# torognes/swarm

Measured on AMD Instinct MI355X. Metric: amplicons/sec clustered (d=1), higher is better.
Workload: dtype u64; 1 GPU; 10000000 synthetic amplicons x 150 bp, d=1 (10000000 per GPU; the metric's own size; configs[1]: configs1); per_gpu_queries=10000000, db_amplicons=10000000, step=swa_d1_index_build + swa_d1_network_device (B1 seam), db and CSR resident in HBM, route=streaming (d1_stream.inc), build=local, neighbour_links=17077441

## Files before the change

swarm_amd/csrc/d1.hip:

```cpp
#include "swa_internal.h"

#include <algorithm>
#include <type_traits>
#include <cstdlib>
#include <memory>
#include <thread>

namespace {

constexpr int kWaves = 4;
constexpr int kThreads = kWaves * 64;
constexpr int kQueueCap = 128;
constexpr uint32_t kEmpty = SWA_NO_AMPLICON;
constexpr size_t kMaxZobristLds = 96 * 1024;

struct alignas(16) swa_task {
  uint64_t hash;
  uint32_t heavy;
  uint32_t code;
};

struct NetArgs {
  const uint64_t * seqs;
  const uint64_t * seq_off;
// ... 591 lines not shown
  if ((threadIdx.x & 63u) == 0u) { ssum[threadIdx.x >> 6] = sum; smax[threadIdx.x >> 6] = mx; sst0[threadIdx.x >> 6] = st0; sst1[threadIdx.x >> 6] = st1; }
  __syncthreads();
  if (threadIdx.x == 0) {
    unsigned long long s = 0, m = 0, a0 = 0, a1 = 0;
    for (int w = 0; w < 16; ++w) { s += ssum[w]; m = m > smax[w] ? m : smax[w]; a0 += sst0[w]; a1 += sst1[w]; }
    out[0] = s; out[1] = m; out[2] = a0; out[3] = a1;
  }
}

__global__ __launch_bounds__(256) void k_seg_bases(const uint32_t * __restrict__ seg_fill, uint32_t nseg,
                                                   unsigned long long * __restrict__ bases) {
  __shared__ unsigned long long part[256];
  const uint32_t chunk = (nseg + 255u) / 256u;
  const uint32_t lo = threadIdx.x * chunk, hi = min(nseg, lo + chunk);
  unsigned long long sum = 0;
  for (uint32_t i = lo; i < hi; ++i) { sum += seg_fill[i]; }
  part[threadIdx.x] = sum;
  __syncthreads();
  if (threadIdx.x == 0) {
    unsigned long long run = 0;
    for (int t = 0; t < 256; ++t) { const unsigned long long v = part[t]; part[t] = run; run += v; }
  }
  __syncthreads();
  unsigned long long at = part[threadIdx.x];
  for (uint32_t i = lo; i < hi; ++i) { bases[i] = at; at += seg_fill[i]; }
}

__global__ __launch_bounds__(256) void k_seg_compact(const uint64_t * __restrict__ edges,
                                                     const uint32_t * __restrict__ seg_fill, uint32_t nseg, uint64_t seg_cap,
                                                     const unsigned long long * __restrict__ bases,
                                                     uint64_t * __restrict__ out, uint64_t cap) {
  for (uint32_t s = blockIdx.x; s < nseg; s += gridDim.x) {
    const uint64_t fill = min((uint64_t)seg_fill[s], seg_cap);
    const uint64_t base = bases[s];
    for (uint64_t i = threadIdx.x; i < fill; i += blockDim.x) {
      if (base + i < cap) { out[base + i] = edges[(uint64_t)s * seg_cap + i]; }
    }
  }
}

#include "d1_fast.inc"
#include "d1_stream.inc"

int grid_for(const swa_ctx * ctx, uint64_t items, int per_block, int max_per_cu) {
  uint64_t blocks = (items + per_block - 1) / per_block;
  const uint64_t cap = (uint64_t)ctx->num_cus * max_per_cu;
  if (blocks > cap) { blocks = cap; }
  if (blocks < 1) { blocks = 1; }
  return (int)blocks;
}

}

void swa_warm_d1(swa_ctx * ctx) {
  hipLaunchKernelGGL(k_table_clear, dim3(1), dim3(64), 0, ctx->stream, static_cast<swa_slot *>(nullptr), (uint64_t)0,
                     static_cast<uint64_t *>(nullptr), (uint64_t)0);
}

int swa_d1_rebuild_table(swa_ctx * ctx, const uint8_t * d_is_member) {
  const uint32_t n = ctx->db.n;
  hipLaunchKernelGGL(k_table_clear, dim3(grid_for(ctx, ctx->table_size, 256, 8)), dim3(256), 0, ctx->stream,
                     static_cast<swa_slot *>(ctx->d_table.ptr), ctx->table_size,
                     static_cast<uint64_t *>(ctx->d_bloom.ptr), ctx->bloom_words);
  hipLaunchKernelGGL(k_table_insert, dim3(grid_for(ctx, n, 256, 8)), dim3(256), 0, ctx->stream,
                     static_cast<const uint64_t *>(ctx->d_seqhash.ptr), n, d_is_member,
                     static_cast<swa_slot *>(ctx->d_table.ptr), ctx->table_size - 1,
                     static_cast<unsigned long long *>(ctx->d_bloom.ptr), ctx->bloom_words - 1,
                     static_cast<const uint64_t *>(ctx->d_patterns.ptr));
  SWA_HIP(ctx, hipGetLastError());
  return SWA_OK;
}


static bool anchored_enabled() {
  const char * e = getenv("SWA_D1_PLAIN");
  return !(e != nullptr && e[0] == '1');
}

static uint32_t anchor_minlen(const swa_ctx * ctx) { return ctx->anchor_a + ctx->anchor_b + 2u * ctx->anchor_w + 1u; }

static bool anchor_applicable(const swa_ctx * ctx) {
  return anchored_enabled() && ctx->db.longest >= kMinAnchoredLen && ctx->db.longest <= 64u * kPrefetchWords * 32u - 64u;
}

static uint32_t line_quads_for(const swa_ctx * ctx) { return ctx->db.longest <= 160u ? 4u : (ctx->db.longest <= 480u ? 8u : 16u); }

static uint32_t anchor_max_nwin(const swa_ctx *) {
  uint32_t cap = 4u;
  if (const char * e = getenv("SWA_D1_ANCHOR_W")) { cap = std::min(4u, std::max(1u, (uint32_t)atoi(e) / 32u)); }
  return cap;
}
static bool windows_search_off() {
  const char * e = getenv("SWA_D1_WINDOWS");
  return e != nullptr && e[0] == '0';
}

static int ensure_db_lengths(swa_ctx * ctx) {
  if (ctx->props_ready) { return SWA_OK; }
  SWA_TRY(swa_reserve(ctx, ctx->d_rank_tmp, std::max<size_t>(ctx->d_rank_tmp.bytes, 64)));
  auto * out = static_cast<uint32_t *>(ctx->d_rank_tmp.ptr);
  SWA_HIP(ctx, hipMemsetAsync(out, 0, 8 * sizeof(uint32_t), ctx->stream));
  hipLaunchKernelGGL(k_db_lengths, dim3(grid_for(ctx, ctx->db.n, 256, 8)), dim3(256), 0, ctx->stream, ctx->db.seqlen, ctx->db.n, out);
  uint32_t host[8] = {};
  SWA_HIP(ctx, hipMemcpyAsync(host, out, sizeof(host), hipMemcpyDeviceToHost, ctx->stream));
  SWA_HIP(ctx, hipStreamSynchronize(ctx->stream));
  ctx->db_shortest = 0xFFFFFFFFu - host[0];
  for (uint32_t c = 0; c <= kWidthClasses; ++c) { ctx->class_pop[c] = host[1 + c]; }
  ctx->props_ready = true;
  return SWA_OK;
}

static ListRegions list_regions(const swa_ctx * ctx, uint64_t * total_items) {
  const uint32_t least[kListKinds] = {2, 5, 9, 17, 33, 65, kPairBigCap + 1u};
  ListRegions r{};
  uint64_t at = 0, upto = 0;
  for (uint32_t c = 0; c < kWidthClasses; ++c) {
    upto += ctx->class_pop[c];
    for (uint32_t k = 0; k < kListKinds; ++k) {
      r.at[c][k] = at;
      uint64_t room = 64;
      constexpr uint64_t per_row_tile = (tiled_item_count(kStreamGroupCap) + kStreamGroupCap / 64u - 1u) / (kStreamGroupCap / 64u);
      if (ctx->class_pop[c] != 0) { room += k + 1 < kListKinds ? std::min<uint64_t>(ctx->class_pop[c], upto / least[k]) : per_row_tile * (upto / 64 + upto / least[k]); }
      at += room;
    }
    r.at[c][kListKinds] = at;
  }
  *total_items = at;
  return r;
}

static int launch_abundance_rank(swa_ctx * ctx) {
  if (ctx->rank_ready) {
    if (ctx->db_unordered) { SWA_HIP(ctx, hipMemsetAsync(static_cast<uint32_t *>(ctx->d_flags.ptr) + 1, 1, sizeof(uint32_t), ctx->stream)); }
    return SWA_OK;
  }
  ctx->rank_ready = true;
  const uint32_t n = ctx->db.n;
  const uint32_t tiles = (n + 255u) / 256u;
  SWA_TRY(swa_reserve(ctx, ctx->d_arank, uint64_t(n) * sizeof(uint32_t)));
  SWA_TRY(swa_reserve(ctx, ctx->d_rank_tmp, uint64_t(tiles) * sizeof(uint32_t)));
  auto * rank = static_cast<uint32_t *>(ctx->d_arank.ptr);
  auto * tile_last = static_cast<uint32_t *>(ctx->d_rank_tmp.ptr);
  hipLaunchKernelGGL(k_abundance_rank, dim3(grid_for(ctx, n, 256, 8)), dim3(256), 0, ctx->stream, ctx->db.abundance, n, rank,
                     static_cast<uint32_t *>(ctx->d_flags.ptr), tile_last);
  hipLaunchKernelGGL(k_abundance_rank_carry, dim3(1), dim3(256), 0, ctx->stream, tile_last, tiles);
  hipLaunchKernelGGL(k_abundance_rank_fill, dim3(grid_for(ctx, n, 256, 8)), dim3(256), 0, ctx->stream, n, rank, tile_last);
  return SWA_OK;
}

__global__ void k_set_flags(uint32_t * flags, uint32_t unserved, uint32_t shortest_code) { flags[3] = unserved; flags[6] = shortest_code; }
__global__ void k_set_guard_made(unsigned long long * guard, uint32_t made0, uint32_t made1) { guard[0] = made0; guard[1] = made1; }

enum { kSbLines = 0, kSbRec = 1, kSbFp = 5, kSbCnt = 8, kSbTile = 10, kSbStart = 12, kSbPartial = 14, kSbScal = 16,
       kSbMembers = 17, kSbOver = 19, kSbKind = 20, kSbLinkA = 22, kSbLinkB = 23, kSbHeavy = 24, kSbMTable = 26, kSbMBloom = 27, kSbSched = 28 };

struct PartPlan { uint32_t levels; uint32_t bits[4]; uint32_t total; };
static PartPlan plan_levels(uint32_t total_bits, uint32_t max_bits = kPartMaxBits) {
  PartPlan p{};
  p.total = std::max(1u, total_bits);
  p.levels = (p.total + max_bits - 1) / max_bits;
  for (uint32_t l = 0; l < p.levels; ++l) { p.bits[l] = p.total / p.levels + (l < p.total % p.levels ? 1u : 0u); }
  return p;
}

struct PartJob {
  uint32_t nidx = 1;
  const unsigned long long * in[kMaxIdx] = {};
  unsigned long long * buf[kMaxIdx][2] = {};
  const uint64_t * cstart0[kMaxIdx] = {};
  uint64_t cstride0[kMaxIdx] = {};
  const uint32_t * csize0[kMaxIdx] = {};
  uint32_t csize_cap = 0, chunks0 = 1;
  bool single0 = true;
  uint64_t max_records = 0, max_tiles0 = 0;
  uint64_t out_cap = 0;
  uint32_t bias = 0, top_bit = 32;
  uint32_t tile = 4096;
  bool hist0_done = false;
  PartPlan plan{};
  uint32_t * out32[kMaxIdx] = {};
  uint32_t * cnt[kMaxIdx] = {}; uint32_t * ctile[kMaxIdx] = {}; uint64_t * starts[kMaxIdx] = {}; uint32_t * partial[kMaxIdx] = {};
  uint32_t * total[kMaxIdx] = {};
  uint64_t starts_stride = 0;
  const unsigned long long * out[kMaxIdx] = {}; const uint64_t * bstart[kMaxIdx] = {};
  uint32_t buckets = 0;
  int last = 0;
};

static void part_scratch(const PartJob & j, uint64_t * cnt, uint64_t * ctile, uint64_t * starts_half, uint64_t * partial) {
  uint64_t chunks = j.chunks0, c_max = 0, t_max = 0, s_max = 0;
  bool single = j.single0;
  for (uint32_t l = 0; l < j.plan.levels; ++l) {
    const uint64_t tiles = (l == 0 ? j.max_tiles0 : j.max_records / j.tile + chunks + 1);
    c_max = std::max(c_max, (tiles << j.plan.bits[l]) + 2);
    t_max = std::max(t_max, chunks + 2 + tiles + 2);
    chunks = (single ? 1 : chunks) << j.plan.bits[l];
    single = false;
    s_max = std::max(s_max, chunks + 2);
  }
  *cnt = c_max; *ctile = t_max; *starts_half = s_max; *partial = c_max / kFlatChunk + 2;
}

struct ClearList { uint32_t * p[8]; uint64_t words[8]; uint32_t n; };
__global__ __launch_bounds__(256) void k_clear_many(const ClearList c) {
  for (uint32_t k = 0; k < c.n; ++k) {
    for (uint64_t i = (uint64_t)blockIdx.x * blockDim.x + threadIdx.x; i < c.words[k]; i += (uint64_t)gridDim.x * blockDim.x) { c.p[k][i] = 0u; }
  }
}
static void clear_add(ClearList & c, void * p, uint64_t bytes) {
  c.p[c.n] = static_cast<uint32_t *>(p); c.words[c.n] = bytes / 4; ++c.n;
}
static int clear_launch(swa_ctx * ctx, const ClearList & c) {
  uint64_t most = 0;
  for (uint32_t k = 0; k < c.n; ++k) { most = std::max(most, c.words[k]); }
  if (c.n == 0 || most == 0) { return SWA_OK; }
  hipLaunchKernelGGL(k_clear_many, dim3(grid_for(ctx, most, 256, 8)), dim3(256), 0, ctx->stream, c);
  SWA_HIP(ctx, hipGetLastError());
  return SWA_OK;
}

static int run_partition(swa_ctx * ctx, PartJob & j) {
  uint64_t chunks = j.chunks0;
  bool single = j.single0;
  uint32_t used_bits = 0;
  const int cu_grid = ctx->num_cus * 8;
  for (uint32_t l = 0; l < j.plan.levels; ++l) {
    const uint32_t bits = j.plan.bits[l];
    used_bits += bits;
    const bool wide = bits > kPartMaxBits;
    const bool hist_done = l == 0 && j.hist0_done;
    const bool low_halves = l + 1 == j.plan.levels && j.out32[0] != nullptr;
    const bool have_form = wide ? (j.tile == 4096 || (j.tile == 8192 && hist_done)) && !low_halves
                                : (j.tile == 2048 && !low_halves) || j.tile == 4096;
    if (!have_form) { return swa_fail_msg(ctx, SWA_E_ARG, "partition: no kernel for this tile and bin count"); }
    PartArgs a{};
    a.single_seg = single ? 1u : 0u; a.bits = bits; a.shift = j.top_bit - used_bits; a.bias = j.bias; a.tile = j.tile;
    a.span = (single && l == 0 && chunks > 1 && j.tile == 4096 && !wide && !hist_done) ? 1u : 0u;
    const uint64_t tiles = (l == 0 ? j.max_tiles0 : j.max_records / j.tile + chunks + 1);
    a.run_bits = tiles >= (uint64_t)cu_grid ? 4u : 0u;
    for (uint32_t i = 0; i < j.nidx; ++i) {
      PartIdx & p = a.p[i];
      p.in = l == 0 ? j.in[i] : j.buf[i][(l - 1) & 1u];
      p.out = j.buf[i][l & 1u];
      p.out32 = low_halves ? j.out32[i] : nullptr;
      p.out_cap = j.out_cap;
      p.cstart = l == 0 ? j.cstart0[i] : j.starts[i] + ((l - 1) & 1u) * j.starts_stride;
      p.cstride = l == 0 ? j.cstride0[i] : 0;
      p.csize = l == 0 ? j.csize0[i] : nullptr;
      p.csize_cap = j.csize_cap;
      p.chunks = (uint32_t)chunks;
      p.ctile = j.ctile[i]; p.cnt = j.cnt[i];
      p.tchunk = j.ctile[i] + chunks + 1; p.tchunk_cap = (uint32_t)std::min<uint64_t>(tiles + 1, 0xFFFFFFFFu);
      p.next_start = j.starts[i] + (l & 1u) * j.starts_stride;
      p.total = j.total[i];
    }
    const dim3 grid_t((unsigned)((std::min<uint64_t>(std::max<uint64_t>(tiles, 1), (uint64_t)cu_grid) + 7) & ~7ull), j.nidx);
    if (chunks > 2048) { hipLaunchKernelGGL(k_part_tiles<1024>, dim3(1, j.nidx), dim3(1024), 0, ctx->stream, a); }
    else { hipLaunchKernelGGL(k_part_tiles<256>, dim3(1, j.nidx), dim3(256), 0, ctx->stream, a); }
    if (hist_done) {  }
    else if (wide) { hipLaunchKernelGGL((k_part_hist<1024, kPartTileMax, 256>), grid_t, dim3(256), 0, ctx->stream, a); }
    else if (a.span != 0u) { hipLaunchKernelGGL((k_part_hist<512, kPartTileMax, 256, true>), grid_t, dim3(256), 0, ctx->stream, a); }
    else { hipLaunchKernelGGL((k_part_hist<512, kPartTileMax, 256>), grid_t, dim3(256), 0, ctx->stream, a); }
    FlatScanArgs f{};
    f.unit_bits = bits;
    for (uint32_t i = 0; i < j.nidx; ++i) { f.v[i] = j.cnt[i]; f.units[i] = j.ctile[i] + chunks; f.partial[i] = j.partial[i]; f.total[i] = j.total[i]; }
    const dim3 grid_f((unsigned)std::min<uint64_t>(((tiles << bits) + 1 + kFlatChunk - 1) / kFlatChunk, (uint64_t)cu_grid), j.nidx);
    hipLaunchKernelGGL(k_flat_sums, grid_f, dim3(256), 0, ctx->stream, f);
    hipLaunchKernelGGL(k_flat_apply, grid_f, dim3(256), 0, ctx->stream, f);
    if (wide && j.tile == 8192) {
      constexpr size_t lds = part_scatter_lds(8192, 1024);
      if (!ctx->part_lds_opt_in) {
        SWA_HIP(ctx, hipFuncSetAttribute(reinterpret_cast<const void *>(&k_part_scatter<0, 8192, 1024, 1024>), hipFuncAttributeMaxDynamicSharedMemorySize, (int)lds));
        ctx->part_lds_opt_in = true;
      }
      hipLaunchKernelGGL((k_part_scatter<0, 8192, 1024, 1024>), grid_t, dim3(1024), lds, ctx->stream, a);
    }
    else if (wide) { hipLaunchKernelGGL((k_part_scatter<0, 4096, 1024, 512>), grid_t, dim3(512), part_scatter_lds(4096, 1024), ctx->stream, a); }
    else if (j.tile == 2048) { hipLaunchKernelGGL((k_part_scatter<0, 2048, 512, 512>), grid_t, dim3(512), part_scatter_lds(2048, 512), ctx->stream, a); }
    else if (a.span != 0u && low_halves) { hipLaunchKernelGGL((k_part_scatter<2, 4096, 512, 512, true>), grid_t, dim3(512), part_scatter_lds(4096, 512), ctx->stream, a); }
    else if (a.span != 0u) { hipLaunchKernelGGL((k_part_scatter<0, 4096, 512, 512, true>), grid_t, dim3(512), part_scatter_lds(4096, 512), ctx->stream, a); }
    else if (low_halves) { hipLaunchKernelGGL((k_part_scatter<2, 4096, 512, 512>), grid_t, dim3(512), part_scatter_lds(4096, 512), ctx->stream, a); }
    else { hipLaunchKernelGGL((k_part_scatter<0, 4096, 512, 512>), grid_t, dim3(512), part_scatter_lds(4096, 512), ctx->stream, a); }
    chunks = (single ? 1 : chunks) << bits;
    single = false;
    hipLaunchKernelGGL(k_part_starts, dim3((unsigned)std::min<uint64_t>((chunks + 256) / 256, (uint64_t)cu_grid), j.nidx), dim3(256), 0, ctx->stream, a);
    SWA_HIP(ctx, hipGetLastError());
  }
  j.buckets = (uint32_t)chunks;
  j.last = (int)((j.plan.levels - 1) & 1u);
  for (uint32_t i = 0; i < j.nidx; ++i) {
    j.out[i] = j.buf[i][j.last];
    j.bstart[i] = j.starts[i] + (uint64_t)j.last * j.starts_stride;
  }
  return SWA_OK;
}

static int ensure_lines(swa_ctx * ctx) {
  const uint32_t lq = line_quads_for(ctx);
  if (ctx->lines_ready && ctx->lines_quads == lq) { return SWA_OK; }
  const uint32_t n = ctx->db.n;
  SWA_TRY(swa_reserve(ctx, ctx->d_stream[kSbLines], (uint64_t)n * lq * 16u + 64u));
  auto * lines = static_cast<uint4 *>(ctx->d_stream[kSbLines].ptr);
  const auto * rank = static_cast<const uint32_t *>(ctx->d_arank.ptr);
  SWA_HIP(ctx, hipMemsetAsync(reinterpret_cast<uint8_t *>(lines) + (uint64_t)n * lq * 16u, 0, 64, ctx->stream));
  swa_t0(ctx, 15);
  const dim3 grid(grid_for(ctx, n, 256, 8));
  if (lq == 4u) { hipLaunchKernelGGL(k_lines_build<4>, grid, dim3(256), 0, ctx->stream, ctx->db.seqs, ctx->db.seq_off, ctx->db.seqlen, rank, n, lines); }
  else if (lq == 8u) { hipLaunchKernelGGL(k_lines_build<8>, grid, dim3(256), 0, ctx->stream, ctx->db.seqs, ctx->db.seq_off, ctx->db.seqlen, rank, n, lines); }
  else { hipLaunchKernelGGL(k_lines_build<16>, grid, dim3(256), 0, ctx->stream, ctx->db.seqs, ctx->db.seq_off, ctx->db.seqlen, rank, n, lines); }
  swa_t1(ctx, 15);
  SWA_HIP(ctx, hipGetLastError());
  ctx->lines_ready = true;
  ctx->lines_quads = lq;
  return SWA_OK;
}

static int build_stream_index(swa_ctx * ctx, uint32_t dup_first, uint32_t dup_count) {
  ctx->anchor_ready = false;
  ctx->stream_index = false;
  ctx->list_counts_ready = false;
  const uint32_t n = ctx->db.n;
  swa_lap(ctx, "(build starts)");
  SWA_TRY(ensure_db_lengths(ctx));
  swa_lap(ctx, "db lengths");
  SWA_TRY(ensure_lines(ctx));
  swa_lap(ctx, "amplicon lines");
  const uint32_t lq = ctx->lines_quads;
  uint64_t item_room = 0;
  const ListRegions regions = list_regions(ctx, &item_room);
  const bool by_rec = ctx->route_rec[0] != nullptr;
  const bool routed = ctx->route_ids[0] != nullptr || by_rec;
  const uint64_t records = routed ? std::max<uint64_t>(std::max(ctx->route_m[0], ctx->route_m[1]), 1) : n;
  const uint32_t target = kG1Target, level_bits = 10u;
  uint32_t total_bits = 1;
  while ((records >> total_bits) > target && total_bits < 3 * kPartMaxBits) { ++total_bits; }
  total_bits = std::min<uint32_t>(total_bits + ctx->stream_extra_bits, 3 * kPartMaxBits);
  const bool keys_hist = !routed;
  PartJob j;
  j.nidx = 2;
  j.plan = total_bits <= level_bits ? plan_levels(total_bits, level_bits) : plan_levels(total_bits);
  j.max_records = records;
  j.out_cap = records + 1;
  const bool one_wide_level = total_bits > kPartMaxBits && j.plan.levels == 1;
  j.tile = one_wide_level ? (keys_hist ? 8192 : 4096) : 2048;
  j.max_tiles0 = records / j.tile + 2;
  j.chunks0 = 1; j.single0 = true; j.top_bit = 32; j.bias = 0;
  uint64_t e_cnt, e_tile, e_start, e_partial;
  part_scratch(j, &e_cnt, &e_tile, &e_start, &e_partial);
  const uint64_t buckets = 1ull << total_bits;
  e_partial = std::max<uint64_t>(e_partial, ((uint64_t)kListsPerIndex * buckets + 1) / kFlatChunk + 2);
  for (int i = 0; i < 2; ++i) {
    for (int h = 0; h < 2; ++h) { SWA_TRY(swa_reserve(ctx, ctx->d_stream[kSbRec + 2 * i + h], (records + 1) * sizeof(uint64_t))); }
    SWA_TRY(swa_reserve(ctx, ctx->d_stream[kSbCnt + i], e_cnt * sizeof(uint32_t)));
    SWA_TRY(swa_reserve(ctx, ctx->d_stream[kSbTile + i], e_tile * sizeof(uint32_t)));
    SWA_TRY(swa_reserve(ctx, ctx->d_stream[kSbStart + i], (2 * e_start + 4) * sizeof(uint64_t)));
    SWA_TRY(swa_reserve(ctx, ctx->d_stream[kSbPartial + i], e_partial * sizeof(uint32_t)));
    SWA_TRY(swa_reserve(ctx, ctx->d_stream[kSbMembers + i], (records + 1) * sizeof(uint32_t)));
    SWA_TRY(swa_reserve(ctx, ctx->d_stream[kSbKind + i], ((uint64_t)kListsPerIndex * buckets + 2) * sizeof(uint32_t)));
    SWA_TRY(swa_reserve(ctx, ctx->d_aitems[i], (item_room + 1) * sizeof(swa_item)));
  }
  SWA_TRY(swa_reserve(ctx, ctx->d_stream[kSbScal], 64 * sizeof(uint64_t)));
  SWA_TRY(swa_reserve(ctx, ctx->d_stream[kSbOver], ((uint64_t)n + 8) & ~3ull));
  SWA_TRY(swa_reserve(ctx, ctx->d_acounters, kCounterWords * sizeof(uint32_t)));
  {
    ClearList c{};
    clear_add(c, ctx->d_acounters.ptr, kCounterWords * sizeof(uint32_t));
    clear_add(c, ctx->d_guard.ptr, 8 * sizeof(uint64_t));
    clear_add(c, ctx->d_stream[kSbOver].ptr, ((uint64_t)n + 8) & ~3ull);
    for (int i = 0; i < 2; ++i) { clear_add(c, static_cast<uint32_t *>(ctx->d_stream[kSbKind + i].ptr) + (uint64_t)kListsPerIndex * buckets, sizeof(uint32_t)); }
    SWA_TRY(clear_launch(ctx, c));
  }
  swa_lap(ctx, "buffers reserved, counters cleared");
  auto * dflags = static_cast<uint32_t *>(ctx->d_flags.ptr);
  auto * scal = static_cast<uint64_t *>(ctx->d_stream[kSbScal].ptr);
  const uint32_t win_a = ctx->anchor_a, win_b = ctx->anchor_b;
  const uint32_t minlen = anchor_minlen(ctx), window_mode = (win_a != 0 || win_b != 0) ? 1u : 0u;

  KeyArgs k{};
  k.lines = static_cast<const uint4 *>(ctx->d_stream[kSbLines].ptr);
  k.line_quads = lq;
  k.seqs = ctx->db.seqs; k.seq_off = ctx->db.seq_off;
  k.n = n;
  for (int i = 0; i < 2; ++i) {
    k.list[i] = routed && !by_rec ? ctx->route_ids[i] : nullptr;
    k.list_count[i] = routed ? ctx->route_m[i] : 0;
    k.rec[i] = static_cast<unsigned long long *>(ctx->d_stream[kSbRec + 2 * i + 1].ptr);
  }
  k.owner_rank = ctx->owner_rank; k.owner_world = ctx->owner_world;
  k.win_a = win_a; k.win_b = win_b; k.minlen = minlen; k.window_mode = window_mode;
  k.nwin = ctx->anchor_w / 32u;
  k.flags = dflags;
  k.guard = static_cast<unsigned long long *>(ctx->d_guard.ptr);
  k.mark_short = (!routed && ctx->owner_world == 1u) ? static_cast<uint8_t *>(ctx->d_stream[kSbOver].ptr) : nullptr;
  if (const char * e = getenv("SWA_D1_GUARD_TEST")) {
    static int builds = 0;
    const bool once = strstr(e, "-once") != nullptr;
    if (!once || builds++ == 0) { k.fault = e[0] == 'm' ? 1u : (e[0] == 'd' ? 2u : 0u); }
  }
  if (routed) {
    hipLaunchKernelGGL(k_set_flags, dim3(1), dim3(1), 0, ctx->stream, dflags,
                       ctx->db_shortest < minlen ? 1u : 0u, 0xFFFFFFFFu - ctx->db_shortest);
  }
  if (by_rec) {
    hipLaunchKernelGGL(k_set_guard_made, dim3(1), dim3(1), 0, ctx->stream, k.guard, ctx->route_m[0], ctx->route_m[1]);
  }
  swa_t0(ctx, 8);
  if (by_rec) {  }
  else if (keys_hist) {
    const uint32_t ntiles = (uint32_t)((records + j.tile - 1) / j.tile);
    for (int i = 0; i < 2; ++i) { k.hist_cnt[i] = static_cast<uint32_t *>(ctx->d_stream[kSbCnt + i].ptr); }
    k.hist_bits = j.plan.bits[0]; k.hist_tile = j.tile; k.hist_ntiles = ntiles;
    k.hist_run_bits = j.max_tiles0 >= (uint64_t)ctx->num_cus * 8 ? 4u : 0u;
    const dim3 hgrid((unsigned)((std::min<uint64_t>(ntiles, (uint64_t)ctx->num_cus * 8) + 7) & ~7ull), 1u);
    hipLaunchKernelGGL(k_keys<true>, hgrid, dim3(256), 0, ctx->stream, k);
    j.hist0_done = true;
  } else {
    const dim3 kgrid((unsigned)grid_for(ctx, records, 256, 8), routed ? 2u : 1u);
    hipLaunchKernelGGL(k_keys<false>, kgrid, dim3(256), 0, ctx->stream, k);
  }
  swa_t1(ctx, 8);
  swa_lap(ctx, "k_keys");

  for (int i = 0; i < 2; ++i) {
    j.buf[i][0] = static_cast<unsigned long long *>(ctx->d_stream[kSbRec + 2 * i].ptr);
    j.buf[i][1] = static_cast<unsigned long long *>(ctx->d_stream[kSbRec + 2 * i + 1].ptr);
    j.in[i] = by_rec ? ctx->route_rec[i] : j.buf[i][1];
    j.cstart0[i] = nullptr; j.cstride0[i] = routed ? ctx->route_m[i] : n;
    j.cnt[i] = static_cast<uint32_t *>(ctx->d_stream[kSbCnt + i].ptr);
    j.ctile[i] = static_cast<uint32_t *>(ctx->d_stream[kSbTile + i].ptr);
    j.starts[i] = static_cast<uint64_t *>(ctx->d_stream[kSbStart + i].ptr);
    j.partial[i] = static_cast<uint32_t *>(ctx->d_stream[kSbPartial + i].ptr);
    j.total[i] = reinterpret_cast<uint32_t *>(scal + 8 + i);
  }
  j.starts_stride = e_start + 2;
  swa_t0(ctx, 9);
  SWA_TRY(run_partition(ctx, j));
  swa_t1(ctx, 9);
  swa_lap(ctx, "key partition");
  if (!ctx->guard_keys_done) {
    auto * gsum = static_cast<unsigned long long *>(ctx->d_guard.ptr) + 16;
    SWA_HIP(ctx, hipMemsetAsync(gsum, 0, 8 * sizeof(uint64_t), ctx->stream));
    GuardDbArgs gd{};
    gd.seqs = ctx->db.seqs; gd.seq_off = ctx->db.seq_off; gd.seqlen = ctx->db.seqlen; gd.n = n;
    for (int i = 0; i < 2; ++i) { gd.list[i] = k.list[i]; gd.list_count[i] = routed ? ctx->route_m[i] : 0; gd.list_rec[i] = by_rec ? ctx->route_rec[i] : nullptr; }
    gd.owner_rank = k.owner_rank; gd.owner_world = k.owner_world; gd.win_a = win_a; gd.win_b = win_b; gd.nwin = k.nwin;
    gd.out = gsum;
    hipLaunchKernelGGL(k_guard_db, dim3((unsigned)grid_for(ctx, records, 256, 8), routed ? 2u : 1u), dim3(256), 0, ctx->stream, gd);
    GuardRecArgs gr{};
    for (int i = 0; i < 2; ++i) { gr.rec[i] = j.out[i]; gr.total[i] = j.total[i]; }
    gr.out = gsum + 3;
    hipLaunchKernelGGL(k_guard_records, dim3((unsigned)grid_for(ctx, records, 256, 8), 2u), dim3(256), 0, ctx->stream, gr);
    ctx->guard_keys_pending = true;
  }

  swa_lap(ctx, "guard: second opinion");
  GroupArgs g{};
  for (int i = 0; i < 2; ++i) {
    GroupIdx & x = g.g[i];
    x.rec = const_cast<unsigned long long *>(j.out[i]);
    x.bstart = j.bstart[i];
    x.buckets = j.buckets;
    x.members = static_cast<uint32_t *>(ctx->d_stream[kSbMembers + i].ptr);
    x.items_tmp = j.buf[i][j.last ^ 1];
    x.kind_cnt = static_cast<uint32_t *>(ctx->d_stream[kSbKind + i].ptr);
  }
  g.pair_big = kPairBigCap; g.group_cap = kStreamGroupCap;
  g.flags = dflags;
  g.guard = static_cast<unsigned long long *>(ctx->d_guard.ptr);
  g.over = static_cast<uint8_t *>(ctx->d_stream[kSbOver].ptr);
  swa_t0(ctx, 10);
  {
    if (!ctx->g1_lds_opt_in) {
      SWA_HIP(ctx, hipFuncSetAttribute(reinterpret_cast<const void *>(&k_group1), hipFuncAttributeMaxDynamicSharedMemorySize, (int)kG1LdsBytes));
      ctx->g1_lds_opt_in = true;
    }
    hipLaunchKernelGGL(k_group1, dim3((unsigned)std::min<uint64_t>(buckets, (uint64_t)ctx->num_cus), 2), dim3(kG1Threads), kG1LdsBytes, ctx->stream, g);
  }
  swa_t1(ctx, 10);

  FlatScanArgs f{};
  ListArgs la{};
  auto * acounters = static_cast<uint32_t *>(ctx->d_acounters.ptr);
  for (int i = 0; i < 2; ++i) {
    f.v[i] = g.g[i].kind_cnt; f.units[i] = nullptr; f.fixed[i] = (uint64_t)kListsPerIndex * buckets + 1;
    f.partial[i] = j.partial[i]; f.total[i] = reinterpret_cast<uint32_t *>(scal + 10 + i);
    ListIdx & x = la.x[i];
    x.items_tmp = g.g[i].items_tmp; x.bstart = g.g[i].bstart; x.kind_pos = g.g[i].kind_cnt; x.buckets = (uint32_t)buckets;
    x.l.items = static_cast<swa_item *>(ctx->d_aitems[i].ptr);
    x.l.region = regions;
    x.l.counters = acounters + kCounterBase + (uint32_t)i * kWidthClasses * 8u;
    x.l.pair_big = g.pair_big;
  }
  const dim3 grid_k((unsigned)std::min<uint64_t>(((uint64_t)kListsPerIndex * buckets + kFlatChunk) / kFlatChunk, (uint64_t)ctx->num_cus * 8), 2);
  hipLaunchKernelGGL(k_flat_sums, grid_k, dim3(256), 0, ctx->stream, f);
  hipLaunchKernelGGL(k_flat_apply, grid_k, dim3(256), 0, ctx->stream, f);
  hipLaunchKernelGGL(k_group_lists, dim3((unsigned)std::min<uint64_t>((buckets + 3) / 4, (uint64_t)ctx->num_cus * 8), 2), dim3(256), 0, ctx->stream, la);
  SWA_HIP(ctx, hipGetLastError());
  swa_lap(ctx, "groups + work lists");
  ctx->list_regions_items = item_room;
  ctx->anchor_ready = true;
  ctx->stream_index = true;
  ctx->guard_index = true;
  return SWA_OK;
}

static int csr_from_chunks(swa_ctx * ctx, uint32_t first, uint32_t count, const unsigned long long * links, const uint64_t * d_cstart, uint64_t cstride,
                           const uint32_t * d_csize, uint32_t chunks, uint32_t csize_cap, uint64_t max_tiles0, uint64_t link_cap,
                           uint64_t * d_offsets, uint32_t * d_neighbours, uint64_t cap) {
  uint32_t nbits = 1;
  while (nbits < 32 && ((uint64_t)1 << nbits) < count) { ++nbits; }
  uint32_t r = std::min<uint32_t>(8, nbits - 1);
  if (nbits - r > 2 * kPartMaxBits) { r = std::min<uint32_t>(kCsrMaxR, nbits - 2 * kPartMaxBits); }
  PartJob j;
  j.nidx = 1;
  j.plan = plan_levels(nbits - r);
  j.max_records = link_cap;
  j.out_cap = link_cap;
  j.tile = 4096;
  j.max_tiles0 = max_tiles0;
  j.chunks0 = chunks; j.single0 = true; j.top_bit = nbits; j.bias = first;
  j.csize_cap = csize_cap;
  uint64_t e_cnt, e_tile, e_start, e_partial;
  part_scratch(j, &e_cnt, &e_tile, &e_start, &e_partial);
  SWA_TRY(swa_reserve(ctx, ctx->d_stream[kSbLinkA], (link_cap + 1) * sizeof(uint64_t)));
  SWA_TRY(swa_reserve(ctx, ctx->d_stream[kSbLinkB], (link_cap + 1) * sizeof(uint64_t)));
  SWA_TRY(swa_reserve(ctx, ctx->d_stream[kSbCnt], e_cnt * sizeof(uint32_t)));
  SWA_TRY(swa_reserve(ctx, ctx->d_stream[kSbTile], e_tile * sizeof(uint32_t)));
  SWA_TRY(swa_reserve(ctx, ctx->d_stream[kSbStart], (2 * e_start + 4) * sizeof(uint64_t)));
  SWA_TRY(swa_reserve(ctx, ctx->d_stream[kSbPartial], e_partial * sizeof(uint32_t)));
  SWA_TRY(swa_reserve(ctx, ctx->d_stream[kSbScal], 64 * sizeof(uint64_t)));
  j.in[0] = links;
  j.buf[0][0] = static_cast<unsigned long long *>(ctx->d_stream[kSbLinkA].ptr);
  j.buf[0][1] = static_cast<unsigned long long *>(ctx->d_stream[kSbLinkB].ptr);
  j.cstart0[0] = d_cstart; j.cstride0[0] = cstride;
  j.csize0[0] = d_csize;
  j.cnt[0] = static_cast<uint32_t *>(ctx->d_stream[kSbCnt].ptr);
  j.ctile[0] = static_cast<uint32_t *>(ctx->d_stream[kSbTile].ptr);
  j.starts[0] = static_cast<uint64_t *>(ctx->d_stream[kSbStart].ptr);
  j.partial[0] = static_cast<uint32_t *>(ctx->d_stream[kSbPartial].ptr);
  auto * extra = static_cast<uint64_t *>(ctx->d_status.ptr) + 48;
  j.total[0] = reinterpret_cast<uint32_t *>(extra + 1);
  j.starts_stride = e_start + 2;
  swa_t0(ctx, 13);
  SWA_TRY(run_partition(ctx, j));
  swa_t1(ctx, 13);
  CsrArgs c{};
  c.links = j.out[0]; c.bstart = j.bstart[0]; c.buckets = j.buckets; c.r = r; c.first = first; c.count = count;
  c.offsets = d_offsets; c.neighbours = d_neighbours; c.cap = d_neighbours != nullptr ? cap : 0;
  SWA_TRY(swa_reserve(ctx, ctx->d_stream[kSbHeavy], ((uint64_t)j.buckets + 2) * sizeof(uint32_t)));
  c.heavy = static_cast<uint32_t *>(ctx->d_stream[kSbHeavy].ptr) + 1;
  c.heavy_count = static_cast<uint32_t *>(ctx->d_stream[kSbHeavy].ptr);
  c.end_copy = extra;
  SWA_HIP(ctx, hipMemsetAsync(c.heavy_count, 0, sizeof(uint32_t), ctx->stream));
  swa_t0(ctx, 14);
  static const int csr_per_cu[2] = {
    [] { int nb = 0; return hipOccupancyMaxActiveBlocksPerMultiprocessor(&nb, k_csr_bucket<8>, 256, 0) == hipSuccess && nb > 0 ? nb : 4; }(),
    [] { int nb = 0; return hipOccupancyMaxActiveBlocksPerMultiprocessor(&nb, k_csr_bucket<9>, 256, 0) == hipSuccess && nb > 0 ? nb : 4; }() };
  const dim3 cgrid((unsigned)std::min<uint64_t>(((uint64_t)j.buckets + 3) / 4, (uint64_t)ctx->num_cus * (uint64_t)csr_per_cu[r <= 8 ? 0 : 1]));
  if (r <= 8) { hipLaunchKernelGGL(k_csr_bucket<8>, cgrid, dim3(256), 0, ctx->stream, c); }
  else { hipLaunchKernelGGL(k_csr_bucket<9>, cgrid, dim3(256), 0, ctx->stream, c); }
  hipLaunchKernelGGL(k_csr_bucket_big, dim3((unsigned)ctx->num_cus * 4), dim3(256), 0, ctx->stream, c);
  swa_t1(ctx, 14);
  SWA_HIP(ctx, hipGetLastError());
  return SWA_OK;
}

static int launch_csr_stream(swa_ctx * ctx, uint32_t first, uint32_t count, uint32_t nseg, uint64_t link_cap, uint64_t * d_offsets,
                             uint32_t * d_neighbours, uint64_t cap) {
  const uint64_t tiles_per_seg = (ctx->seg_cap + 4096 - 1) / 4096;
  return csr_from_chunks(ctx, first, count, static_cast<const unsigned long long *>(ctx->d_edges.ptr), nullptr, ctx->seg_cap,
                         static_cast<const uint32_t *>(ctx->d_seg_fill.ptr), nseg, (uint32_t)std::min<uint64_t>(ctx->seg_cap, 0xFFFFFFFFu),
                         (uint64_t)nseg * tiles_per_seg + 2, link_cap, d_offsets, d_neighbours, cap);
}

#define SWA_PAIR_CASE(KERNEL, P, WW, NN) \
  if (pass == P && width == WW && nwin == NN) { hipLaunchKernelGGL((KERNEL<P, WW, NN>), dim3(grid), dim3(kThreads), 0, ctx->stream, a); return SWA_OK; }
#define SWA_PAIR_WIDTH(KERNEL, WW) \
  SWA_PAIR_CASE(KERNEL, 0, WW, 1) SWA_PAIR_CASE(KERNEL, 1, WW, 1) SWA_PAIR_CASE(KERNEL, 0, WW, 2) SWA_PAIR_CASE(KERNEL, 1, WW, 2)
#define SWA_PAIR_CASES(KERNEL) \
  SWA_PAIR_WIDTH(KERNEL, 5) SWA_PAIR_WIDTH(KERNEL, 8) SWA_PAIR_WIDTH(KERNEL, 15) SWA_PAIR_WIDTH(KERNEL, 21) \
  SWA_PAIR_CASE(KERNEL, 0, 15, 4) SWA_PAIR_CASE(KERNEL, 1, 15, 4) SWA_PAIR_CASE(KERNEL, 0, 21, 4) SWA_PAIR_CASE(KERNEL, 1, 21, 4)
#define SWA_PAIR_CASE_DYN(KERNEL, P, WW, NN) \
  if (pass == P && width == WW && nwin == NN) { \
    const int bytes = (int)PairLayout<WW>::kDynamicBytes; \
    constexpr uint32_t bit_ = 1u << (P + (WW == 21 ? 2 : 0) + (NN == 2 ? 4 : (NN == 4 ? 8 : 0))); \
    if (bytes != 0 && (ctx->pair_lds_opt_in & bit_) == 0u) {      \
      SWA_HIP(ctx, hipFuncSetAttribute(reinterpret_cast<const void *>(&KERNEL<P, WW, NN>), hipFuncAttributeMaxDynamicSharedMemorySize, bytes)); \
      ctx->pair_lds_opt_in |= bit_; \
    } \
    hipLaunchKernelGGL((KERNEL<P, WW, NN>), dim3(grid), dim3(kThreads), (size_t)bytes, ctx->stream, a); return SWA_OK; }
#define SWA_PAIR_WIDTH_DYN(KERNEL, WW) \
  SWA_PAIR_CASE_DYN(KERNEL, 0, WW, 1) SWA_PAIR_CASE_DYN(KERNEL, 1, WW, 1) SWA_PAIR_CASE_DYN(KERNEL, 0, WW, 2) SWA_PAIR_CASE_DYN(KERNEL, 1, WW, 2)
static int launch_group_pairs(swa_ctx * ctx, int pass, int width, int nwin, int grid, const AnchorArgs & a) {
  SWA_PAIR_WIDTH_DYN(k_d1_group_pairs, 5) SWA_PAIR_WIDTH_DYN(k_d1_group_pairs, 8) SWA_PAIR_WIDTH_DYN(k_d1_group_pairs, 15) SWA_PAIR_WIDTH_DYN(k_d1_group_pairs, 21)
  SWA_PAIR_CASE_DYN(k_d1_group_pairs, 0, 15, 4) SWA_PAIR_CASE_DYN(k_d1_group_pairs, 1, 15, 4) SWA_PAIR_CASE_DYN(k_d1_group_pairs, 0, 21, 4) SWA_PAIR_CASE_DYN(k_d1_group_pairs, 1, 21, 4)
  return swa_fail_msg(ctx, SWA_E_ARG, "pair kernels: no kernel for this record / window width");
}
static int launch_pairs_tiled(swa_ctx * ctx, int pass, int width, int nwin, int grid, const AnchorArgs & a) {
  SWA_PAIR_CASES(k_d1_pairs_tiled)
  return swa_fail_msg(ctx, SWA_E_ARG, "pair kernels: no kernel for this record / window width");
}

static int pair_blocks_per_cu(swa_ctx * ctx, uint32_t cls) {
  int & c = ctx->pair_blocks[cls];
  if (c == 0) {
    int nb = 0;
    const hipError_t e = cls == 0 ? hipOccupancyMaxActiveBlocksPerMultiprocessor(&nb, k_d1_group_pairs<0, 5, 1>, kThreads, 0)
                       : cls == 1 ? hipOccupancyMaxActiveBlocksPerMultiprocessor(&nb, k_d1_group_pairs<0, 8, 1>, kThreads, 0)
                       : cls == 2 ? hipOccupancyMaxActiveBlocksPerMultiprocessor(&nb, k_d1_group_pairs<0, 15, 1>, kThreads, PairLayout<15>::kDynamicBytes)
                                  : hipOccupancyMaxActiveBlocksPerMultiprocessor(&nb, k_d1_group_pairs<0, 21, 1>, kThreads, PairLayout<21>::kDynamicBytes);
    c = (e == hipSuccess && nb >= 1) ? std::min(nb, 8) : (cls <= 1u ? 4 : (cls == 2u ? 2 : 1));
  }
  return c;
}

static uint32_t seg_count(const swa_ctx * ctx) { return (uint32_t)ctx->num_cus * 8u * kWaves; }

static int launch_network_anchored(swa_ctx * ctx, int ncb, uint32_t first, uint32_t count) {
  auto * acounters = static_cast<uint32_t *>(ctx->d_acounters.ptr);
  SWA_TRY(swa_reserve(ctx, ctx->d_afallback, (2ull * count + 16) * sizeof(swa_fallback)));
  ClearList clears{};
  clear_add(clears, ctx->d_stats.ptr, 16 * sizeof(uint64_t));
  clear_add(clears, static_cast<uint64_t *>(ctx->d_guard.ptr) + 8, 8 * sizeof(uint64_t));
  clear_add(clears, acounters, kCounterBase * sizeof(uint32_t));
  clear_add(clears, ctx->d_seg_fill.ptr, 3ull * seg_count(ctx) * sizeof(uint32_t));
  uint32_t shard_bits = 6;
  while (shard_bits > 0 && (1u << shard_bits) > (uint32_t)ctx->num_cus) { --shard_bits; }
  {
    const uint64_t bytes = ((2ull * kWidthClasses) << shard_bits) * kSchedStride * sizeof(uint32_t);
    SWA_TRY(swa_reserve(ctx, ctx->d_stream[kSbSched], bytes));
    clear_add(clears, ctx->d_stream[kSbSched].ptr, bytes);
  }
  SWA_TRY(clear_launch(ctx, clears));
  const bool zlds = 4ull * ctx->zobrist_len * sizeof(uint64_t) <= kMaxZobristLds;
  const uint32_t maxwords = (ctx->db.longest + 31u) >> 5;
  swa_t0(ctx, 3);
  const bool window_mode = ctx->anchor_a != 0 || ctx->anchor_b != 0;
  uint64_t item_room = 0;
  const ListRegions regions = list_regions(ctx, &item_room);
  if (item_room != ctx->list_regions_items) { return swa_fail_msg(ctx, SWA_E_ARG, "d=1 network: the work lists in place were laid out for another database"); }
  const int nwin = (int)(ctx->anchor_w / 32u);
  for (int pass = 0; pass < 2; ++pass) {
    swa_t0(ctx, 11 + pass);
    AnchorArgs a{};
    a.pass = pass;
    a.no_cluster_breaking = ncb;
    a.first = first; a.count = count;
    a.edges = static_cast<uint64_t *>(ctx->d_edges.ptr);
    a.seg_cap = ctx->seg_cap;
    a.seg_fill = static_cast<uint32_t *>(ctx->d_seg_fill.ptr);
    a.minlen = anchor_minlen(ctx);
    a.win_word = ctx->anchor_a / 32u;
    a.win_word_b = ctx->anchor_b / 32u;
    a.window_mode = window_mode ? 1u : 0u;
    a.seg_staged = static_cast<uint32_t *>(ctx->d_seg_fill.ptr) + (uint64_t)(1 + pass) * seg_count(ctx);
    a.guard = static_cast<unsigned long long *>(ctx->d_guard.ptr);
    a.flags = static_cast<uint32_t *>(ctx->d_flags.ptr);
    a.shard_bits = shard_bits;
    a.ids = static_cast<const uint32_t *>(ctx->d_stream[kSbMembers + pass].ptr);
    a.lines = static_cast<const uint4 *>(ctx->d_stream[kSbLines].ptr);
    a.line_quads = ctx->lines_quads;
    a.pair_items = static_cast<const swa_item *>(ctx->d_aitems[pass].ptr);
    for (uint32_t cls = 0; cls < kWidthClasses; ++cls) {
      if (ctx->class_pop[cls] == 0) { continue; }
      const int width = width_words(cls);
      if (nwin == 4 && width < 15) { return swa_fail_msg(ctx, SWA_E_ARG, "pair kernels: 128-nt windows with sequences of 256 nt or less"); }
      const uint32_t pc = (uint32_t)pass * kWidthClasses + cls;
      for (uint32_t k = 0; k <= kPairClasses; ++k) { a.pair_region[k] = regions.at[cls][k]; }
      a.pair_counters = acounters + kCounterBase + pc * 8u;
      a.items = a.pair_items + regions.at[cls][kPairClasses + 1u];
      a.item_count = a.pair_counters + kPairClasses + 1u;
      a.sched_big = acounters + 8 + 2 * pc;
      a.sched_tiled = acounters + 9 + 2 * pc;
      a.sched_wide = static_cast<uint32_t *>(ctx->d_stream[kSbSched].ptr) + ((uint64_t)pc << shard_bits) * kSchedStride;
      const uint32_t * have = ctx->list_counts_ready ? ctx->list_counts + pc * 8u : nullptr;
      bool any_pairs = have == nullptr;
      for (uint32_t k = 0; k <= kPairClasses && have != nullptr; ++k) { any_pairs = any_pairs || have[k] != 0u; }
      const int pgrid = ctx->num_cus * pair_blocks_per_cu(ctx, cls);
      {
        uint64_t bundles = 0;
        for (uint32_t k = 0; k < kPairClasses && have != nullptr; ++k) { bundles += ((uint64_t)have[k] + (16u >> k) - 1u) >> (4u - k); }
        const uint64_t waves = (uint64_t)pgrid * 4u;
        a.batch = have == nullptr || bundles >= 16u * waves ? 4u : (bundles >= 8u * waves ? 2u : 1u);
      }
      if (any_pairs) { SWA_TRY(launch_group_pairs(ctx, pass, width, nwin, pgrid, a)); }
      if (have == nullptr || have[kPairClasses + 1u] != 0u) { SWA_TRY(launch_pairs_tiled(ctx, pass, width, nwin, ctx->num_cus * (cls <= 1u ? 8 : 4), a)); }
    }
    swa_t1(ctx, 11 + pass);
    SWA_HIP(ctx, hipGetLastError());
  }
  const bool use_member_table = ctx->member_index && !ctx->full_index;
  if (ctx->full_index || ctx->member_index) {
    hipLaunchKernelGGL(k_stream_fallback, dim3(grid_for(ctx, count, 256, 8)), dim3(256), 0, ctx->stream, ctx->db.seqlen, first, count,
                       static_cast<const uint8_t *>(ctx->d_stream[kSbOver].ptr), static_cast<swa_fallback *>(ctx->d_afallback.ptr), acounters + 2,
                       ctx->owner_rank, ctx->owner_world, ctx->db.seqs, ctx->db.seq_off, anchor_minlen(ctx));
  }
  NetArgs f{};
  f.seqs = ctx->db.seqs; f.seq_off = ctx->db.seq_off; f.seqlen = ctx->db.seqlen; f.abundance = ctx->db.abundance;
  f.zobrist = static_cast<const uint64_t *>(ctx->d_zobrist.ptr);
  f.zlen = ctx->zobrist_len; f.maxwords = maxwords;
  f.table = static_cast<const swa_slot *>(use_member_table ? ctx->d_stream[kSbMTable].ptr : ctx->d_table.ptr);
  f.tmask = (use_member_table ? ctx->mtable_size : ctx->table_size) - 1;
  f.bloom = static_cast<const uint64_t *>(use_member_table ? ctx->d_stream[kSbMBloom].ptr : ctx->d_bloom.ptr);
  f.bmask = (use_member_table ? ctx->mbloom_words : ctx->bloom_words) - 1;
  f.patterns = static_cast<const uint64_t *>(ctx->d_patterns.ptr);
  f.no_cluster_breaking = ncb;
  f.first = first; f.count = count;
  f.edges = static_cast<uint64_t *>(ctx->d_edges.ptr);
  f.seg_cap = ctx->seg_cap;
  f.seg_fill = static_cast<uint32_t *>(ctx->d_seg_fill.ptr);
  f.fallback = static_cast<const swa_fallback *>(ctx->d_afallback.ptr);
  f.fallback_count = acounters + 2;
  f.aux = static_cast<const swa_aux *>(ctx->d_aux.ptr);
  f.owner_rank = 0; f.owner_world = 1;
  f.window_mode = window_mode ? 1u : 0u; f.win_word = ctx->anchor_a / 32u; f.anchor_w = ctx->anchor_w;
  const size_t flds = sizeof(uint64_t) * ((zlds ? 4ull * ctx->zobrist_len : 0ull) + 1024ull +
                                          kWaves * ((size_t)(maxwords + 2u) + kQueueCap + kQueueCap / 2));
  const int fgrid = grid_for(ctx, count, kWaves, 8);
  if (!ctx->full_index && !ctx->member_index) {  }
  else if (zlds) { hipLaunchKernelGGL((k_d1_probe<true, 2>), dim3(fgrid), dim3(kThreads), flds, ctx->stream, f); }
  else { hipLaunchKernelGGL((k_d1_probe<false, 2>), dim3(fgrid), dim3(kThreads), flds, ctx->stream, f); }
  swa_t1(ctx, 3);
  SWA_HIP(ctx, hipGetLastError());
  return SWA_OK;
}
// ... 2 lines not shown
  const uint32_t n = ctx->db.n;
  ctx->zobrist_len = ctx->db.longest + 2;
  SWA_TRY(swa_reserve(ctx, ctx->d_seqhash, uint64_t(n) * sizeof(uint64_t)));
  SWA_TRY(swa_reserve(ctx, ctx->d_aux, uint64_t(n) * sizeof(swa_aux)));
  if (ctx->zobrist_resident != ctx->zobrist_len) {
    std::vector<uint64_t> zob;
    swa_zobrist_table(ctx->zobrist_len, zob);
    SWA_TRY(swa_reserve(ctx, ctx->d_zobrist, zob.size() * sizeof(uint64_t)));
    SWA_HIP(ctx, hipMemcpyAsync(ctx->d_zobrist.ptr, zob.data(), zob.size() * sizeof(uint64_t), hipMemcpyHostToDevice, ctx->stream));
    SWA_HIP(ctx, hipStreamSynchronize(ctx->stream));
    ctx->zobrist_resident = ctx->zobrist_len;
  }
  return SWA_OK;
}

static int launch_seqhash(swa_ctx * ctx, const uint8_t * only = nullptr) {
  const uint32_t n = ctx->db.n;
  const size_t zbytes = 4ull * ctx->zobrist_len * sizeof(uint64_t);
  const bool zlds = zbytes <= kMaxZobristLds;
  swa_t0(ctx, 0);
  const int hgrid = grid_for(ctx, n, 256, 8);
  if (zlds) {
    hipLaunchKernelGGL(k_seqhash<true>, dim3(hgrid), dim3(256), zbytes, ctx->stream, ctx->db.seqs, ctx->db.seq_off,
                       ctx->db.seqlen, static_cast<const uint64_t *>(ctx->d_zobrist.ptr), ctx->zobrist_len, n,
                       static_cast<uint64_t *>(ctx->d_seqhash.ptr), static_cast<swa_aux *>(ctx->d_aux.ptr), ctx->anchor_w, only);
  } else {
    hipLaunchKernelGGL(k_seqhash<false>, dim3(hgrid), dim3(256), 0, ctx->stream, ctx->db.seqs, ctx->db.seq_off,
                       ctx->db.seqlen, static_cast<const uint64_t *>(ctx->d_zobrist.ptr), ctx->zobrist_len, n,
                       static_cast<uint64_t *>(ctx->d_seqhash.ptr), static_cast<swa_aux *>(ctx->d_aux.ptr), ctx->anchor_w, only);
  }
  SWA_HIP(ctx, hipGetLastError());
  swa_t1(ctx, 0);
  return SWA_OK;
}

int swa_hash_sequences(swa_ctx * ctx) {
  SWA_TRY(prepare_hashing(ctx));
  return launch_seqhash(ctx);
}

extern "C" int swa_d1_index_build(swa_ctx * ctx, int * has_duplicates) {
  if (ctx == nullptr) { return SWA_E_ARG; }
  return swa_d1_index_build_range(ctx, 0, ctx->db.n, has_duplicates);
}

static int ensure_full_index(swa_ctx * ctx) {
  if (ctx->full_index) { return SWA_OK; }
  SWA_TRY(swa_reserve(ctx, ctx->d_table, ctx->table_size * sizeof(swa_slot)));
  SWA_TRY(swa_reserve(ctx, ctx->d_bloom, ctx->bloom_words * sizeof(uint64_t)));
  SWA_TRY(swa_hash_sequences(ctx));
  swa_t0(ctx, 1);
  SWA_TRY(swa_d1_rebuild_table(ctx, nullptr));
  swa_t1(ctx, 1);
  ctx->full_index = true;
  return SWA_OK;
}

static int choose_anchor_windows(swa_ctx * ctx) {
  ctx->anchor_a = ctx->anchor_b = 0;
  ctx->anchor_w = 32;
  SWA_TRY(ensure_db_lengths(ctx));
  const uint32_t shortest = ctx->db_shortest;
  const uint32_t n = ctx->db.n;
  const uint32_t max_nwin = anchor_max_nwin(ctx);
  ctx->anchor_w = 32u * anchor_nwin_for(shortest, 0u, max_nwin);
  if (windows_search_off()) { return SWA_OK; }
  const uint32_t stride = std::max<uint32_t>(1u, n / 65536u);
  const uint32_t samples = (n + stride - 1) / stride;
  const size_t slots = (size_t)2 * kSampleCandidates * kSampleSlots;
  SWA_TRY(swa_reserve(ctx, ctx->d_akeys[0], std::max<size_t>(ctx->d_akeys[0].bytes, slots * sizeof(uint64_t))));
  SWA_TRY(swa_reserve(ctx, ctx->d_acounts[0], std::max<size_t>(ctx->d_acounts[0].bytes, (slots + 16) * sizeof(uint32_t))));
  auto * keys = static_cast<unsigned long long *>(ctx->d_akeys[0].ptr);
  auto * counts = static_cast<uint32_t *>(ctx->d_acounts[0].ptr);
  uint32_t * stats = counts + slots;
  SWA_HIP(ctx, hipMemsetAsync(keys, 0xFF, slots * sizeof(uint64_t), ctx->stream));
  SWA_HIP(ctx, hipMemsetAsync(counts, 0, (slots + 16) * sizeof(uint32_t), ctx->stream));
  hipLaunchKernelGGL(k_anchor_sample, dim3(grid_for(ctx, samples, 256, 8)), dim3(256), 0, ctx->stream, ctx->db.seqs, ctx->db.seq_off,
                     ctx->db.seqlen, n, stride, keys, counts, stats, shortest, max_nwin);
  hipLaunchKernelGGL(k_sample_mass, dim3(grid_for(ctx, slots, 256, 8)), dim3(256), 0, ctx->stream, counts, stride, stats + 4);
  uint32_t host[8] = {};
  SWA_HIP(ctx, hipMemcpyAsync(host, stats, sizeof(host), hipMemcpyDeviceToHost, ctx->stream));
  SWA_HIP(ctx, hipStreamSynchronize(ctx->stream));
  for (uint32_t c = 0; c < kSampleCandidates; ++c) {
    const bool few_short = host[c] <= samples / 64u || c == 0;
    if (host[4 + c] <= samples / 64u && few_short) {
      ctx->anchor_a = ctx->anchor_b = 32u * c;
      ctx->anchor_w = 32u * anchor_nwin_for(shortest, 32u * c, max_nwin);
      return SWA_OK;
    }
    if (!few_short) { break; }
  }
  return SWA_OK;
}

static int ensure_anchor_windows(swa_ctx * ctx) {
  if (!ctx->windows_ready) {
    SWA_TRY(choose_anchor_windows(ctx));
    ctx->windows_chosen = ctx->anchor_a;
    ctx->windows_w = ctx->anchor_w;
    ctx->windows_ready = true;
  }
  ctx->anchor_a = ctx->anchor_b = ctx->windows_chosen;
  ctx->anchor_w = ctx->windows_w;
  return SWA_OK;
}


static int build_member_index(swa_ctx * ctx, uint32_t dup_first, uint32_t dup_count) {
  ctx->member_index = false;
  const uint32_t n = ctx->db.n;
  SWA_TRY(prepare_hashing(ctx));
  SWA_TRY(launch_seqhash(ctx, static_cast<const uint8_t *>(ctx->d_stream[kSbOver].ptr)));
  uint64_t slots = 1024;
  while (slots < 2ull * ctx->over_mass) { slots <<= 1; }
  const uint64_t words = std::max<uint64_t>(slots >> 3, 1);
  SWA_TRY(swa_reserve(ctx, ctx->d_stream[kSbMTable], slots * sizeof(swa_slot)));
  SWA_TRY(swa_reserve(ctx, ctx->d_stream[kSbMBloom], words * sizeof(uint64_t)));
  auto * table = static_cast<swa_slot *>(ctx->d_stream[kSbMTable].ptr);
  auto * bloom = static_cast<uint64_t *>(ctx->d_stream[kSbMBloom].ptr);
  swa_t0(ctx, 1);
  hipLaunchKernelGGL(k_table_clear, dim3(grid_for(ctx, slots, 256, 8)), dim3(256), 0, ctx->stream, table, slots, bloom, words);
  hipLaunchKernelGGL(k_table_insert, dim3(grid_for(ctx, n, 256, 8)), dim3(256), 0, ctx->stream, static_cast<const uint64_t *>(ctx->d_seqhash.ptr), n,
                     static_cast<const uint8_t *>(ctx->d_stream[kSbOver].ptr), table, slots - 1, reinterpret_cast<unsigned long long *>(bloom), words - 1,
                     static_cast<const uint64_t *>(ctx->d_patterns.ptr));
  swa_t1(ctx, 1);
  swa_t0(ctx, 2);
  if (dup_count != 0) {
    hipLaunchKernelGGL(k_dup_check, dim3(grid_for(ctx, dup_count, 256, 8)), dim3(256), 0, ctx->stream, ctx->db.seqs, ctx->db.seq_off, ctx->db.seqlen,
                       static_cast<const uint64_t *>(ctx->d_seqhash.ptr), dup_first, dup_count, table, slots - 1, static_cast<uint32_t *>(ctx->d_flags.ptr));
  }
  swa_t1(ctx, 2);
  SWA_HIP(ctx, hipGetLastError());
  ctx->mtable_size = slots;
  ctx->mbloom_words = words;
  ctx->member_index = true;
  return SWA_OK;
}

static int build_owned_index(swa_ctx * ctx, uint32_t first, uint32_t count, bool * needs_table, uint32_t * dups, uint32_t * oversized_mass = nullptr,
                             uint32_t * shortest = nullptr) {
  const uint32_t n = ctx->db.n;
  auto * dflags = static_cast<uint32_t *>(ctx->d_flags.ptr);
  swa_lap(ctx, "(owned index starts)");
  SWA_TRY(launch_abundance_rank(ctx));
  swa_lap(ctx, "abundance ranks");
  const uint32_t dup_first = ctx->owner_world > 1 ? 0u : first, dup_count = ctx->owner_world > 1 ? n : count;
  swa_t0(ctx, 7);
  SWA_TRY(build_stream_index(ctx, dup_first, dup_count));
  swa_t1(ctx, 7);
  auto * status = static_cast<uint32_t *>(ctx->h_status);
  SWA_HIP(ctx, hipMemcpyAsync(status, ctx->d_status.ptr, 512 * sizeof(uint32_t), hipMemcpyDeviceToHost, ctx->stream));
  SWA_HIP(ctx, hipStreamSynchronize(ctx->stream));
  const uint32_t * flags = status;
  *dups = flags[0];
  memcpy(ctx->list_counts, status + 256 + kCounterBase, sizeof(ctx->list_counts));
  ctx->list_counts_ready = true;
  if (oversized_mass != nullptr) { *oversized_mass = flags[5]; }
  if (shortest != nullptr) { *shortest = 0xFFFFFFFFu - flags[6]; }
  if (flags[2] != 0) {
    if (ctx->stream_extra_bits >= 8) { return swa_fail_msg(ctx, SWA_E_DEVICE, "streaming index build: partition still too coarse"); }
    ctx->stream_extra_bits += 2;
    SWA_HIP(ctx, hipMemsetAsync(dflags, 0, 16 * sizeof(uint32_t), ctx->stream));
    return build_owned_index(ctx, first, count, needs_table, dups, oversized_mass, shortest);
  }
  if (flags[1] != 0) { ctx->db_unordered = true; }
  *needs_table = flags[1] != 0 || flags[3] != 0 || flags[4] != 0;
  ctx->only_oversized = flags[1] == 0 && (flags[4] != 0 || flags[3] != 0) &&
                        (flags[3] == 0 || (ctx->owner_world == 1u && ctx->route_ids[0] == nullptr && ctx->route_rec[0] == nullptr));
  ctx->over_mass = flags[5];
  return SWA_OK;
}

extern "C" int swa_d1_index_build_range(swa_ctx * ctx, uint32_t first, uint32_t count, int * has_duplicates) {
  if (ctx == nullptr) { return SWA_E_ARG; }
  if (ctx->db.n == 0) { return swa_fail_msg(ctx, SWA_E_ARG, "swa_d1_index_build: no database"); }
  if (first > ctx->db.n || count > ctx->db.n - first) { return swa_fail_msg(ctx, SWA_E_ARG, "swa_d1_index_build_range: bad range"); }
  SWA_HIP(ctx, hipSetDevice(ctx->device));
  const uint32_t n = ctx->db.n;
  ctx->index_first = first; ctx->index_count = count; ctx->index_routed = ctx->route_ids[0] != nullptr || ctx->route_rec[0] != nullptr;
  ctx->d1_ready = false;
  ctx->csr_ready = false;
  ctx->anchor_ready = false;
  ctx->full_index = false;
  ctx->member_index = false;
  ctx->anchor_a = ctx->anchor_b = 0;
  for (int slot : {0, 1, 2, 7, 8, 9, 10, 15}) { ctx->ev_used[slot] = false; }
  ctx->table_size = swa_hashtable_size(n);
  const uint64_t bloom_bytes = ctx->table_size < 8 ? 8 : ctx->table_size;
  ctx->bloom_words = bloom_bytes >> 3;

  if (!ctx->patterns_resident) {
    std::vector<uint64_t> pat;
    swa_bloom_patterns(1024, 8, pat);
    SWA_TRY(swa_reserve(ctx, ctx->d_patterns, pat.size() * sizeof(uint64_t)));
    SWA_HIP(ctx, hipMemcpyAsync(ctx->d_patterns.ptr, pat.data(), pat.size() * sizeof(uint64_t), hipMemcpyHostToDevice, ctx->stream));
    SWA_HIP(ctx, hipStreamSynchronize(ctx->stream));
    ctx->patterns_resident = true;
  }
  SWA_TRY(swa_reserve(ctx, ctx->d_flags, 16 * sizeof(uint32_t)));
  SWA_TRY(swa_reserve(ctx, ctx->d_stats, 16 * sizeof(uint64_t)));
  SWA_TRY(swa_reserve(ctx, ctx->d_guard, 24 * sizeof(uint64_t)));
  SWA_HIP(ctx, hipMemsetAsync(ctx->d_status.ptr, 0, 64 + 128 + 16 * sizeof(uint64_t), ctx->stream));
  ctx->guard_index = false;
  ctx->anchor_w = 32;
  ctx->anchor_usable = anchor_applicable(ctx);

  bool owned_ok = false;
  uint32_t group_dups = 0;
  if (ctx->anchor_usable) {
    bool needs_table = false;
    uint32_t mass = 0, shortest = 0;
    swa_lap(ctx, "(index build: before the windows)");
    SWA_TRY(ensure_anchor_windows(ctx));
    swa_lap(ctx, "anchor windows");
    const uint32_t sampled = ctx->anchor_a;
    const bool routed = ctx->route_ids[0] != nullptr || ctx->route_rec[0] != nullptr;
    SWA_TRY(build_owned_index(ctx, first, count, &needs_table, &group_dups, &mass, &shortest));
    if (!routed && ctx->owner_world == 1 && needs_table && mass > n / 64u && !windows_search_off()) {
      uint32_t best = sampled, best_mass = mass;
      for (uint32_t w = sampled + 32u; 2u * w + kMinAnchoredLen <= shortest && w <= 96u; w += 32u) {
        ctx->anchor_a = ctx->anchor_b = w;
        ctx->anchor_w = 32;
        SWA_HIP(ctx, hipMemsetAsync(ctx->d_flags.ptr, 0, 16 * sizeof(uint32_t), ctx->stream));
        uint32_t m = 0;
        SWA_TRY(build_owned_index(ctx, first, count, &needs_table, &group_dups, &m));
        if (m < best_mass) { best_mass = m; best = w; }
        if (m <= n / 64u) { break; }
      }
      if (ctx->anchor_a != best) {
        ctx->anchor_a = ctx->anchor_b = best;
        ctx->anchor_w = best == sampled ? ctx->windows_w : 32u;
        SWA_HIP(ctx, hipMemsetAsync(ctx->d_flags.ptr, 0, 16 * sizeof(uint32_t), ctx->stream));
        SWA_TRY(build_owned_index(ctx, first, count, &needs_table, &group_dups));
      }
    }
    ctx->windows_chosen = ctx->anchor_a;
    ctx->windows_w = ctx->anchor_w;
    owned_ok = !needs_table;
    if (!owned_ok && ctx->only_oversized) {
      SWA_TRY(build_member_index(ctx, ctx->owner_world > 1 ? 0u : first, ctx->owner_world > 1 ? n : count));
      owned_ok = true;
      auto * mirror = static_cast<uint32_t *>(ctx->h_status);
      SWA_HIP(ctx, hipMemcpyAsync(mirror, ctx->d_flags.ptr, sizeof(uint32_t), hipMemcpyDeviceToHost, ctx->stream));
      SWA_HIP(ctx, hipStreamSynchronize(ctx->stream));
      group_dups = mirror[0];
    }
    if (!owned_ok) { SWA_HIP(ctx, hipMemsetAsync(ctx->d_flags.ptr, 0, 16 * sizeof(uint32_t), ctx->stream)); }
  }
  uint32_t flag = group_dups;
  if (!owned_ok) {
    SWA_TRY(ensure_full_index(ctx));
    swa_t0(ctx, 2);
    if (count > 0) {
      hipLaunchKernelGGL(k_dup_check, dim3(grid_for(ctx, count, 256, 8)), dim3(256), 0, ctx->stream, ctx->db.seqs, ctx->db.seq_off,
                         ctx->db.seqlen, static_cast<const uint64_t *>(ctx->d_seqhash.ptr), first, count,
                         static_cast<const swa_slot *>(ctx->d_table.ptr), ctx->table_size - 1,
                         static_cast<uint32_t *>(ctx->d_flags.ptr));
    }
    SWA_HIP(ctx, hipGetLastError());
    swa_t1(ctx, 2);
    if (ctx->anchor_usable) {
      SWA_TRY(launch_abundance_rank(ctx));
      SWA_HIP(ctx, hipGetLastError());
    }
    uint32_t flags[2] = {0, 0};
    SWA_HIP(ctx, hipMemcpyAsync(flags, ctx->d_flags.ptr, sizeof(flags), hipMemcpyDeviceToHost, ctx->stream));
    SWA_HIP(ctx, hipStreamSynchronize(ctx->stream));
    flag |= flags[0];
    if (flags[1] != 0) { ctx->anchor_usable = false; ctx->db_unordered = true; }
  }
  ctx->d1_ready = true;
  if (has_duplicates != nullptr) { *has_duplicates = flag != 0 ? 1 : 0; }
  if (flag != 0) {
    return swa_fail_msg(ctx, SWA_E_DUPLICATES, "some fasta entries have identical sequences");
  }
  return SWA_OK;
}

extern "C" uint32_t swa_d1_anchor_width(const swa_ctx * ctx) { return ctx != nullptr ? ctx->anchor_w : 0; }

extern "C" uint64_t swa_d1_table_size(const swa_ctx * ctx) { return ctx != nullptr ? ctx->table_size : 0; }

extern "C" int swa_d1_anchor_windows(const swa_ctx * ctx, uint32_t * out2) {
  if (ctx == nullptr || out2 == nullptr) { return SWA_E_ARG; }
  out2[0] = ctx->anchor_a; out2[1] = ctx->anchor_b;
  return SWA_OK;
}

static size_t network_lds_bytes(const swa_ctx * ctx, bool zlds) {
  const uint32_t maxwords = (ctx->db.longest + 31u) >> 5;
  const size_t per_wave = (size_t)(maxwords + 2u) + kQueueCap + kQueueCap / 2;
  return sizeof(uint64_t) * ((zlds ? 4ull * ctx->zobrist_len : 0ull) + 1024ull + kWaves * per_wave);
}

static int launch_network(swa_ctx * ctx, int ncb, uint32_t first, uint32_t count) {
  NetArgs a{};
  a.seqs = ctx->db.seqs; a.seq_off = ctx->db.seq_off; a.seqlen = ctx->db.seqlen; a.abundance = ctx->db.abundance;
  a.zobrist = static_cast<const uint64_t *>(ctx->d_zobrist.ptr);
  a.zlen = ctx->zobrist_len;
  a.maxwords = (ctx->db.longest + 31u) >> 5;
  a.table = static_cast<const swa_slot *>(ctx->d_table.ptr);
  a.tmask = ctx->table_size - 1;
  a.bloom = static_cast<const uint64_t *>(ctx->d_bloom.ptr);
  a.bmask = ctx->bloom_words - 1;
  a.patterns = static_cast<const uint64_t *>(ctx->d_patterns.ptr);
  a.no_cluster_breaking = ncb;
  a.first = first; a.count = count;
  a.edges = static_cast<uint64_t *>(ctx->d_edges.ptr);
  a.seg_cap = ctx->seg_cap;
  a.seg_fill = static_cast<uint32_t *>(ctx->d_seg_fill.ptr);
  a.owner_rank = ctx->owner_rank; a.owner_world = ctx->owner_world;
  a.anchor_w = 32;
  SWA_HIP(ctx, hipMemsetAsync(ctx->d_stats.ptr, 0, 16 * sizeof(uint64_t), ctx->stream));
  const bool zlds = 4ull * ctx->zobrist_len * sizeof(uint64_t) <= kMaxZobristLds;
  const size_t lds = network_lds_bytes(ctx, zlds);
  const int grid = grid_for(ctx, count, kWaves, 8);
  swa_t0(ctx, 3);
  if (zlds) { hipLaunchKernelGGL((k_d1_probe<true, 0>), dim3(grid), dim3(kThreads), lds, ctx->stream, a); }
  else { hipLaunchKernelGGL((k_d1_probe<false, 0>), dim3(grid), dim3(kThreads), lds, ctx->stream, a); }
  swa_t1(ctx, 3);
  SWA_HIP(ctx, hipGetLastError());
  return SWA_OK;
}

static int guard_check(swa_ctx * ctx, const uint64_t * g, const uint64_t * got) {
  char msg[256];
  if (g[10] != 0) {
    snprintf(msg, sizeof(msg), "d=1 guard: %llu member(s) filed under an anchor key that is not theirs", (unsigned long long)g[10]);
    return swa_fail_msg(ctx, SWA_E_INTERNAL, msg);
  }
  if (ctx->stream_index && ctx->guard_keys_pending) {
    ctx->guard_keys_pending = false;
    for (int i = 0; i < 2; ++i) {
      if (g[16 + i] != g[19 + i]) {
        snprintf(msg, sizeof(msg), "d=1 guard: the %s derived from the amplicon lines are not the ones the packed database gives (%016llx / %016llx)",
                 i == 0 ? "prefix-side key records" : "suffix-side key records", (unsigned long long)g[19 + i],
                 (unsigned long long)g[16 + i]);
        return swa_fail_msg(ctx, SWA_E_INTERNAL, msg);
      }
    }
    ctx->guard_keys_done = true;
  }
  if (ctx->stream_index && ctx->guard_index) {
    for (int i = 0; i < 2; ++i) {
      if (g[i] != g[2 + i] + g[4 + i] + g[6 + i]) {
        snprintf(msg, sizeof(msg), "d=1 guard: index %d has %llu key records but %llu + %llu + %llu grouped members", i, (unsigned long long)g[i],
                 (unsigned long long)g[2 + i], (unsigned long long)g[4 + i], (unsigned long long)g[6 + i]);
        return swa_fail_msg(ctx, SWA_E_INTERNAL, msg);
      }
      if (got[2 + i] != g[2 + i]) {
        snprintf(msg, sizeof(msg), "d=1 guard: pass %d staged %llu members of %llu listed", i, (unsigned long long)got[2 + i], (unsigned long long)g[2 + i]);
        return swa_fail_msg(ctx, SWA_E_INTERNAL, msg);
      }
    }
  }
  return SWA_OK;
}
static int csr_check(swa_ctx * ctx, uint64_t csr_end, uint32_t links_sorted, uint64_t n_edges) {
  if (csr_end != n_edges || (uint64_t)links_sorted != (n_edges & 0xFFFFFFFFull)) {
    char msg[256];
    snprintf(msg, sizeof(msg), "d=1 guard: %llu links found, %u sorted, CSR ends at %llu", (unsigned long long)n_edges, links_sorted, (unsigned long long)csr_end);
    return swa_fail_msg(ctx, SWA_E_INTERNAL, msg);
  }
  return SWA_OK;
}

static int network_run(swa_ctx * ctx, int no_cluster_breaking, uint32_t first, uint32_t count, uint64_t * d_offsets,
                       uint32_t * d_neighbours, uint64_t * d_edge_list, uint64_t cap, uint64_t * total) {
  SWA_HIP(ctx, hipSetDevice(ctx->device));
  const uint32_t nseg = (uint32_t)ctx->num_cus * 8u * kWaves;
  SWA_TRY(swa_reserve(ctx, ctx->d_seg_fill, 3ull * nseg * sizeof(uint32_t)));
  SWA_TRY(swa_reserve(ctx, ctx->d_guard, 24 * sizeof(uint64_t)));
  if (ctx->seg_cap == 0) {
    ctx->seg_cap = 512;
    while (ctx->seg_cap < 8ull * count / nseg) { ctx->seg_cap <<= 1; }
    const char * env_cap = getenv("SWA_D1_SEG_CAP");
    if (env_cap != nullptr && atoi(env_cap) > 0) { ctx->seg_cap = (uint64_t)atoi(env_cap); }
  }
  uint64_t n_edges = 0;
  uint64_t stream_link_cap = 0;
  bool clean = false;
  bool twins = false;
  for (int attempt = 0; attempt < 8 && !clean; ++attempt) {
    SWA_TRY(swa_reserve(ctx, ctx->d_edges, uint64_t(nseg) * ctx->seg_cap * sizeof(uint64_t)));
    if (!ctx->anchor_usable) { SWA_HIP(ctx, hipMemsetAsync(ctx->d_seg_fill.ptr, 0, 3ull * nseg * sizeof(uint32_t), ctx->stream)); }
    if (ctx->anchor_usable) {
      if (!(ctx->anchor_ready && ctx->stream_index)) {
        swa_t0(ctx, 7);
        SWA_TRY(launch_abundance_rank(ctx));
        SWA_HIP(ctx, hipMemsetAsync(static_cast<uint32_t *>(ctx->d_flags.ptr) + 2, 0, 5 * sizeof(uint32_t), ctx->stream));
        SWA_TRY(build_stream_index(ctx, 0, 0));
        swa_t1(ctx, 7);
        if (!ctx->full_index) {
          uint32_t fl[6] = {};
          SWA_HIP(ctx, hipMemcpyAsync(fl, ctx->d_flags.ptr, sizeof(fl), hipMemcpyDeviceToHost, ctx->stream));
          SWA_HIP(ctx, hipStreamSynchronize(ctx->stream));
          ctx->member_index = false;
          if (fl[3] != 0 || fl[4] != 0) { SWA_TRY(ensure_full_index(ctx)); }
        }
      }
      SWA_TRY(launch_network_anchored(ctx, no_cluster_breaking, first, count));
    }
    else {
      SWA_TRY(ensure_full_index(ctx));
      SWA_TRY(launch_network(ctx, no_cluster_breaking, first, count));
    }
    hipLaunchKernelGGL(k_seg_reduce, dim3(1), dim3(1024), 0, ctx->stream, static_cast<const uint32_t *>(ctx->d_seg_fill.ptr),
                       nseg, static_cast<unsigned long long *>(ctx->d_stats.ptr) + 8);
    const bool check_unserved = ctx->anchor_usable && !ctx->full_index && !ctx->member_index;
    swa_t0(ctx, 4);
    if (d_edge_list != nullptr) {
      SWA_TRY(swa_reserve(ctx, ctx->d_seg_base, uint64_t(nseg) * sizeof(uint64_t)));
      hipLaunchKernelGGL(k_seg_bases, dim3(1), dim3(256), 0, ctx->stream, static_cast<const uint32_t *>(ctx->d_seg_fill.ptr), nseg,
                         static_cast<unsigned long long *>(ctx->d_seg_base.ptr));
      hipLaunchKernelGGL(k_seg_compact, dim3(std::min<uint32_t>(nseg, (uint32_t)ctx->num_cus * 8u)), dim3(256), 0, ctx->stream,
                         static_cast<const uint64_t *>(ctx->d_edges.ptr), static_cast<const uint32_t *>(ctx->d_seg_fill.ptr),
                         nseg, ctx->seg_cap, static_cast<const unsigned long long *>(ctx->d_seg_base.ptr), d_edge_list, cap);
    } else {
      stream_link_cap = std::max<uint64_t>(std::max<uint64_t>(cap, stream_link_cap), 2ull * count + 1024);
      SWA_TRY(launch_csr_stream(ctx, first, count, nseg, stream_link_cap, d_offsets, d_neighbours, cap));
    }
    SWA_HIP(ctx, hipGetLastError());
    swa_t1(ctx, 4);
    auto * status = static_cast<uint64_t *>(ctx->h_status);
    SWA_HIP(ctx, hipMemcpyAsync(status, ctx->d_status.ptr, 64 * sizeof(uint64_t), hipMemcpyDeviceToHost, ctx->stream));
    uint32_t * unserved_at = reinterpret_cast<uint32_t *>(status + 64);
    *unserved_at = 0;
    if (check_unserved) {
      SWA_HIP(ctx, hipMemcpyAsync(unserved_at, static_cast<uint32_t *>(ctx->d_acounters.ptr) + 2, sizeof(uint32_t), hipMemcpyDeviceToHost, ctx->stream));
    }
    SWA_HIP(ctx, hipStreamSynchronize(ctx->stream));
    const uint32_t unserved = *unserved_at;
    const uint64_t * got = status + 8 + 8;
    const uint64_t * guard = status + 24;
    const uint32_t anchor_overflow = reinterpret_cast<const uint32_t *>(status)[2];
    const uint64_t csr_end = status[48];
    const uint32_t links_sorted = (uint32_t)status[49];
    const bool guarded = ctx->anchor_usable;
    n_edges = got[0];
    if (guarded && anchor_overflow != 0) {
      ctx->stream_extra_bits = std::min<uint32_t>(ctx->stream_extra_bits + 2, 8);
      ctx->anchor_ready = false;
      continue;
    }
    if (check_unserved && unserved != 0) {
      SWA_TRY(ensure_full_index(ctx));
      continue;
    }
    if (d_edge_list == nullptr && got[1] <= ctx->seg_cap && n_edges > stream_link_cap) {
      stream_link_cap = n_edges + 1024;
      continue;
    }
    if (got[1] <= ctx->seg_cap) {
      clean = true;
      if (guarded) { SWA_TRY(guard_check(ctx, guard, got)); }
      if (d_edge_list == nullptr) { SWA_TRY(csr_check(ctx, csr_end, links_sorted, n_edges)); }
      twins = guarded && reinterpret_cast<const uint32_t *>(status)[0] != 0u;
      break;
    }
    while (ctx->seg_cap < 2 * got[1]) { ctx->seg_cap <<= 1; }
  }
  if (!clean) {
    return swa_fail_msg(ctx, SWA_E_DEVICE, "swa_d1_network: per-wave link segments still overflowed after 8 attempts");
  }
  *total = n_edges;
  if (twins) { return swa_fail_msg(ctx, SWA_E_DUPLICATES, "some fasta entries have identical sequences"); }
  if (n_edges > cap) { return swa_fail_msg(ctx, SWA_E_CAPACITY, "swa_d1_network: neighbour buffer too small"); }
  return SWA_OK;
}

static int network_run_guarded(swa_ctx * ctx, int no_cluster_breaking, uint32_t first, uint32_t count, uint64_t * d_offsets,
                               uint32_t * d_neighbours, uint64_t * d_edge_list, uint64_t cap, uint64_t * total) {
  const int rc = network_run(ctx, no_cluster_breaking, first, count, d_offsets, d_neighbours, d_edge_list, cap, total);
  if (rc != SWA_E_INTERNAL || ctx->index_routed) { return rc; }
  const std::string first_msg = ctx->err;
  fprintf(stderr, "swarm-amd: %s; rebuilding the index from the packed database and repeating the step\n", first_msg.c_str());
  ++ctx->guard_retries;
  ctx->lines_ready = ctx->props_ready = ctx->windows_ready = ctx->rank_ready = false;
  ctx->anchor_ready = ctx->stream_index = ctx->member_index = ctx->full_index = false;
  ctx->guard_index = ctx->guard_keys_done = ctx->guard_keys_pending = false;
  ctx->stream_extra_bits = 0;
  int dup = 0;
  const int rb = swa_d1_index_build_range(ctx, ctx->index_first, ctx->index_count, &dup);
  if (rb != SWA_OK && rb != SWA_E_DUPLICATES) { return rb; }
  const int again = network_run(ctx, no_cluster_breaking, first, count, d_offsets, d_neighbours, d_edge_list, cap, total);
  if (again == SWA_E_INTERNAL) { ctx->err = first_msg + "; after a rebuild: " + ctx->err; }
  return again;
}

extern "C" int swa_d1_guard_retries(const swa_ctx * ctx) { return ctx != nullptr ? (int)ctx->guard_retries : 0; }

extern "C" int swa_d1_network_device(swa_ctx * ctx, int no_cluster_breaking, uint32_t first, uint32_t count,
                                     uint64_t * d_offsets, uint32_t * d_neighbours, uint64_t cap, uint64_t * total) {
  if (ctx == nullptr) { return SWA_E_ARG; }
  if (!ctx->d1_ready) { return swa_fail_msg(ctx, SWA_E_ARG, "swa_d1_network: call swa_d1_index_build first"); }
  if (count == 0 || (uint64_t)first + count > ctx->db.n || d_offsets == nullptr || total == nullptr ||
      (d_neighbours == nullptr && cap != 0)) {
    return swa_fail_msg(ctx, SWA_E_ARG, "swa_d1_network: bad range or null buffer");
  }
  return network_run_guarded(ctx, no_cluster_breaking, first, count, d_offsets, d_neighbours, nullptr, cap, total);
}

extern "C" int swa_d1_network_edges_device(swa_ctx * ctx, int no_cluster_breaking, uint32_t first, uint32_t count,
                                           uint64_t * d_edge_list, uint64_t cap, uint64_t * total) {
  if (ctx == nullptr) { return SWA_E_ARG; }
  if (!ctx->d1_ready) { return swa_fail_msg(ctx, SWA_E_ARG, "swa_d1_network: call swa_d1_index_build first"); }
  if (count == 0 || (uint64_t)first + count > ctx->db.n || d_edge_list == nullptr || total == nullptr) {
    return swa_fail_msg(ctx, SWA_E_ARG, "swa_d1_network_edges: bad range or null buffer");
  }
  return network_run_guarded(ctx, no_cluster_breaking, first, count, nullptr, nullptr, d_edge_list, cap, total);
}

int swa_d1_csr_from_lists(swa_ctx * ctx, const unsigned long long * d_links, const uint64_t * starts, const uint64_t * counts, uint32_t lists,
                          uint64_t * d_offsets, uint32_t * d_neighbours, uint64_t cap) {
  SWA_HIP(ctx, hipSetDevice(ctx->device));
  const uint32_t n = ctx->db.n;
  uint64_t all = 0, tiles = 2;
  std::vector<uint64_t> h_start(lists);
  std::vector<uint32_t> h_size(lists);
  for (uint32_t r = 0; r < lists; ++r) {
    if (counts[r] > 0xFFFFFFFFull) { return swa_fail_msg(ctx, SWA_E_CAPACITY, "swa_d1_csr_from_lists: a list of more than 2^32 links"); }
    h_start[r] = starts[r]; h_size[r] = (uint32_t)counts[r];
    all += counts[r]; tiles += (counts[r] + 4095) / 4096;
  }
  SWA_TRY(swa_reserve(ctx, ctx->d_seg_base, ((uint64_t)lists * 3 / 2 + 2) * sizeof(uint64_t)));
  auto * d_start = static_cast<uint64_t *>(ctx->d_seg_base.ptr);
  auto * d_size = reinterpret_cast<uint32_t *>(d_start + lists);
  SWA_HIP(ctx, hipMemcpyAsync(d_start, h_start.data(), lists * sizeof(uint64_t), hipMemcpyHostToDevice, ctx->stream));
  SWA_HIP(ctx, hipMemcpyAsync(d_size, h_size.data(), lists * sizeof(uint32_t), hipMemcpyHostToDevice, ctx->stream));
  SWA_HIP(ctx, hipStreamSynchronize(ctx->stream));
  return csr_from_chunks(ctx, 0, n, d_links, d_start, 0, d_size, lists, 0xFFFFFFFFu, tiles, all + 1, d_offsets, d_neighbours, cap);
}

extern "C" int swa_d1_route_slice(swa_ctx * ctx, uint32_t first, uint32_t count, uint32_t world, uint32_t * d_ids, uint64_t cap,
                                  uint32_t * d_counts) {
  if (ctx == nullptr) { return SWA_E_ARG; }
  if (ctx->db.n == 0) { return swa_fail_msg(ctx, SWA_E_ARG, "swa_d1_route_slice: no database"); }
  if (first > ctx->db.n || count > ctx->db.n - first) { return swa_fail_msg(ctx, SWA_E_ARG, "swa_d1_route_slice: bad range"); }
  if (world == 0 || world > kRouteMaxWorld || d_ids == nullptr || d_counts == nullptr || cap == 0) {
    return swa_fail_msg(ctx, SWA_E_ARG, "swa_d1_route_slice: bad argument (1..64 ranks)");
  }
  SWA_HIP(ctx, hipSetDevice(ctx->device));
  SWA_TRY(swa_reserve(ctx, ctx->d_flags, 16 * sizeof(uint32_t)));
  SWA_TRY(ensure_anchor_windows(ctx));
  SWA_HIP(ctx, hipMemsetAsync(d_counts, 0, (2ull * world + 1) * sizeof(uint32_t), ctx->stream));
  if (count != 0) {
    hipLaunchKernelGGL(k_anchor_route, dim3(grid_for(ctx, (count + kRoutePerThread - 1) / kRoutePerThread, 256, 8)), dim3(256), 0, ctx->stream,
                       ctx->db.seqs, ctx->db.seq_off, ctx->db.seqlen, first, count, world, ctx->anchor_a, ctx->anchor_b, ctx->anchor_w / 32u, d_ids, cap,
                       d_counts);
  }
  SWA_HIP(ctx, hipGetLastError());
  SWA_HIP(ctx, hipStreamSynchronize(ctx->stream));
  return SWA_OK;
}

extern "C" int swa_d1_index_build_routed(swa_ctx * ctx, const uint32_t * d_ids_prefix, uint32_t n_prefix, const uint32_t * d_ids_suffix,
                                         uint32_t n_suffix, int * has_duplicates) {
  if (ctx == nullptr) { return SWA_E_ARG; }
  if (ctx->db.n == 0) { return swa_fail_msg(ctx, SWA_E_ARG, "swa_d1_index_build_routed: no database"); }
  if (ctx->owner_world <= 1) { return swa_fail_msg(ctx, SWA_E_ARG, "swa_d1_index_build_routed: call swa_d1_set_ownership(rank, world > 1) first"); }
  if ((n_prefix != 0 && d_ids_prefix == nullptr) || (n_suffix != 0 && d_ids_suffix == nullptr)) { return swa_fail_msg(ctx, SWA_E_ARG, "swa_d1_index_build_routed: null list"); }
  SWA_HIP(ctx, hipSetDevice(ctx->device));
  SWA_TRY(ensure_db_lengths(ctx));
  static const uint32_t nothing = 0;
  ctx->route_ids[0] = n_prefix != 0 ? d_ids_prefix : &nothing; ctx->route_m[0] = n_prefix;
  ctx->route_ids[1] = n_suffix != 0 ? d_ids_suffix : &nothing; ctx->route_m[1] = n_suffix;
  const int rc = swa_d1_index_build_range(ctx, 0, ctx->db.n, has_duplicates);
  ctx->route_ids[0] = ctx->route_ids[1] = nullptr;
  ctx->route_m[0] = ctx->route_m[1] = 0;
  return rc;
}

extern "C" int swa_d1_route_slice_records(swa_ctx * ctx, uint32_t first, uint32_t count, uint32_t world, uint64_t * d_records, uint64_t cap,
                                          uint32_t * d_counts) {
  if (ctx == nullptr) { return SWA_E_ARG; }
  if (ctx->db.n == 0) { return swa_fail_msg(ctx, SWA_E_ARG, "swa_d1_route_slice_records: no database"); }
  if (first > ctx->db.n || count > ctx->db.n - first) { return swa_fail_msg(ctx, SWA_E_ARG, "swa_d1_route_slice_records: bad range"); }
  if (world == 0 || world > kRouteMaxWorld || d_records == nullptr || d_counts == nullptr || cap == 0) {
    return swa_fail_msg(ctx, SWA_E_ARG, "swa_d1_route_slice_records: bad argument (1..64 ranks)");
  }
  SWA_HIP(ctx, hipSetDevice(ctx->device));
  SWA_TRY(swa_reserve(ctx, ctx->d_flags, 16 * sizeof(uint32_t)));
  SWA_TRY(ensure_anchor_windows(ctx));
  SWA_HIP(ctx, hipMemsetAsync(d_counts, 0, (2ull * world + 1) * sizeof(uint32_t), ctx->stream));
  if (count != 0) {
    hipLaunchKernelGGL(k_anchor_route_records, dim3(grid_for(ctx, (count + 3) / 4, 256, 8)), dim3(256), 0, ctx->stream,
                       ctx->db.seqs, ctx->db.seq_off, ctx->db.seqlen, first, count, world, ctx->anchor_a, ctx->anchor_b, ctx->anchor_w / 32u,
                       reinterpret_cast<unsigned long long *>(d_records), cap, d_counts);
  }
  SWA_HIP(ctx, hipGetLastError());
// ... 437 lines not shown
```

swarm_amd/csrc/d1_stream.inc:

```

constexpr uint32_t kPartTileMax = 4096;
constexpr uint32_t kPartMaxBits = 9;
constexpr unsigned long long kRecAbsent = ~0ull;
constexpr uint32_t kMaxIdx = 2;
constexpr uint32_t kStreamGroupCap = 4096;

template <int LQ>
__global__ __launch_bounds__(256) void k_lines_build(const uint64_t * __restrict__ seqs, const uint64_t * __restrict__ seq_off,
                                                     const uint32_t * __restrict__ seqlen, const uint32_t * __restrict__ rank, uint32_t n,
                                                     uint4 * __restrict__ lines) {
  constexpr uint32_t C = 2u * LQ - 1u;
  for (uint32_t i = blockIdx.x * blockDim.x + threadIdx.x; i < n; i += gridDim.x * blockDim.x) {
    const uint32_t len = seqlen[i];
    const uint64_t * s = seqs + seq_off[i];
    const uint32_t nw = (len + 31u) >> 5;
    uint32_t d[4 * LQ];
    d[0] = len; d[1] = rank[i];
#pragma unroll
    for (uint32_t k = 0; k < C; ++k) {
      const uint64_t w = k < nw ? s[k] : 0ull;
      d[2 + 2 * k] = (uint32_t)w; d[3 + 2 * k] = (uint32_t)(w >> 32);
    }
#pragma unroll
    for (uint32_t q = 0; q < (uint32_t)LQ; ++q) { lines[(uint64_t)i * LQ + q] = make_uint4(d[4 * q], d[4 * q + 1], d[4 * q + 2], d[4 * q + 3]); }
// ... 285 lines not shown
    for (uint32_t k = 0; k < 8u; ++k) {
      const uint32_t c = base + threadIdx.x * 8u + k;
      v[k] = c < p.chunks ? (a.span != 0u ? part_chunk_size(p, c) : (part_chunk_size(p, c) + a.tile - 1u) / a.tile) : 0u;
    }
#pragma unroll
    for (uint32_t k = 0; k < 8u; ++k) { mine += v[k]; }
    uint64_t total;
    uint64_t run = carry + block_exclusive_scan_of<THREADS>(mine, smem, total);
#pragma unroll
    for (uint32_t k = 0; k < 8u; ++k) {
      const uint32_t c = base + threadIdx.x * 8u + k;
      if (c < p.chunks) {
        p.ctile[c] = (uint32_t)run;
        if (v[k] != 0u && a.span != 0u) {
          const uint32_t r32 = (uint32_t)run;
          const uint32_t first = tile_pow2 ? (r32 + a.tile - 1u) >> tile_shift : (r32 + a.tile - 1u) / a.tile;
          const uint32_t n = (tile_pow2 ? (r32 + v[k] + a.tile - 1u) >> tile_shift : (r32 + v[k] + a.tile - 1u) / a.tile) - first;
          if (n <= 4u) {
#pragma unroll
            for (uint32_t i = 0; i < 4u; ++i) { if (i < n && first + i < p.tchunk_cap) { p.tchunk[first + i] = c; } }
          }
        }
      }
      run += v[k];
    }
    carry += total;
  }
  if (threadIdx.x == 0) {
    if (a.span != 0u) { carry = ((uint32_t)carry + a.tile - 1u) / a.tile; }
    p.ctile[p.chunks] = (uint32_t)carry;
    p.cnt[carry << a.bits] = 0u;
  }
}

__device__ __forceinline__ uint32_t part_chunk_of(const uint32_t * ctile, uint32_t chunks, uint32_t t) {
  uint32_t lo = 0, hi = chunks;
  while (lo < hi) { const uint32_t mid = (lo + hi) >> 1; if (ctile[mid] <= t) { lo = mid + 1u; } else { hi = mid; } }
  return lo - 1u;
}

__device__ __forceinline__ uint64_t part_flat(const PartArgs & a, const PartIdx & p, uint32_t c, uint32_t t, uint32_t b) {
  if (a.single_seg != 0u) { return (uint64_t)b * p.ctile[p.chunks] + t; }
  const uint32_t t0 = p.ctile[c], nt = p.ctile[c + 1] - t0;
  return ((uint64_t)t0 << a.bits) + (uint64_t)b * nt + (t - t0);
}

struct PartTile { uint32_t c, count; uint64_t first; };

__device__ __forceinline__ PartTile part_tile(const PartIdx & p, uint32_t tile_records, uint32_t t, uint32_t * sh) {
  if (threadIdx.x == 0) {
    sh[0] = part_chunk_of(p.ctile, p.chunks, t);
  }
  __syncthreads();
  PartTile r;
  r.c = sh[0];
  const uint32_t within = (t - p.ctile[r.c]) * tile_records;
  r.first = (p.cstart != nullptr ? p.cstart[r.c] : (p.csize != nullptr ? (uint64_t)r.c * p.cstride : 0ull)) + within;
  r.count = min(tile_records, part_chunk_size(p, r.c) - within);
  return r;
}

constexpr uint32_t kSpanFast = 4;
constexpr uint32_t kSpanRound = 256;
struct SpanLds { uint32_t c_lo, n, count, q0; uint64_t shift[kSpanFast]; uint32_t before[kSpanRound + 1]; };
__device__ __forceinline__ uint64_t part_chunk_base(const PartIdx & p, uint32_t c) {
  return p.cstart != nullptr ? p.cstart[c] : (p.csize != nullptr ? (uint64_t)c * p.cstride : 0ull);
}
template <uint32_t PER, uint32_t THREADS, typename Take>
__device__ __forceinline__ uint32_t part_span(const PartIdx & p, uint32_t tile_records, uint32_t t, SpanLds & s, Take take) {
  if (threadIdx.x == 0) {
    const uint32_t last = p.chunks - 1u;
    const uint32_t total = p.ctile[last] + part_chunk_size(p, last);
    const uint32_t q0 = t * tile_records, q1 = min(q0 + tile_records, total) - 1u;
    const auto chunk_at = [&](uint32_t tile, uint32_t q) -> uint32_t {
      const uint32_t c = tile < p.tchunk_cap ? p.tchunk[tile] : 0xFFFFFFFFu;
      if (c < p.chunks && p.ctile[c] <= q && q < (c + 1u < p.chunks ? p.ctile[c + 1u] : total)) { return c; }
      return part_chunk_of(p.ctile, p.chunks, q);
    };
    const uint32_t c_lo = chunk_at(t, q0);
    const uint32_t c_hi = q1 + 1u < total ? chunk_at(t + 1u, q1 + 1u) : part_chunk_of(p.ctile, p.chunks, q1);
    s.c_lo = c_lo; s.n = c_hi - c_lo + 1u; s.count = q1 - q0 + 1u; s.q0 = q0;
  }
  __syncthreads();
  const uint32_t n = s.n, count = s.count, q0 = s.q0, c_lo = s.c_lo;
  if (n <= kSpanFast) {
    if (threadIdx.x < n) {
      const uint32_t before = p.ctile[c_lo + threadIdx.x];
      s.before[threadIdx.x] = before;
      s.shift[threadIdx.x] = part_chunk_base(p, c_lo + threadIdx.x) - before;
    }
    __syncthreads();
    const uint32_t b1 = n > 1u ? s.before[1] : 0xFFFFFFFFu, b2 = n > 2u ? s.before[2] : 0xFFFFFFFFu, b3 = n > 3u ? s.before[3] : 0xFFFFFFFFu;
#pragma unroll
    for (uint32_t k = 0; k < PER; ++k) {
      const uint32_t j = k * THREADS + threadIdx.x, q = q0 + j;
      const uint32_t i = (q >= b1 ? 1u : 0u) + (q >= b2 ? 1u : 0u) + (q >= b3 ? 1u : 0u);
      if (j < count) { take(k, s.shift[i] + q); }
    }
    return count;
  }
  for (uint32_t r0 = 0; r0 < n; r0 += kSpanRound) {
    const uint32_t m = min(kSpanRound, n - r0);
    if (r0 != 0u) { __syncthreads(); }
    for (uint32_t i = threadIdx.x; i <= m; i += THREADS) { s.before[i] = r0 + i < n ? p.ctile[c_lo + r0 + i] : 0xFFFFFFFFu; }
    __syncthreads();
    const uint32_t from = s.before[0], upto = s.before[m];
#pragma unroll
    for (uint32_t k = 0; k < PER; ++k) {
      const uint32_t j = k * THREADS + threadIdx.x, q = q0 + j;
      if (j < count && q >= from && q < upto) {
        uint32_t lo = 0, hi = m;
        while (lo < hi) { const uint32_t mid = (lo + hi) >> 1; if (s.before[mid] <= q) { lo = mid + 1u; } else { hi = mid; } }
        take(k, part_chunk_base(p, c_lo + r0 + lo - 1u) + (q - s.before[lo - 1u]));
      }
    }
  }
  return count;
}

template <uint32_t BINS, uint32_t TILE, uint32_t THREADS, bool SPAN = false>
__global__ __launch_bounds__(THREADS) void k_part_hist(const PartArgs a) {
  __shared__ uint32_t hist[BINS];
  __shared__ uint32_t sh[1];
  __shared__ typename std::conditional<SPAN, SpanLds, uint32_t>::type span;
  const PartIdx & p = a.p[blockIdx.y];
  const uint32_t bins = 1u << a.bits;
  const uint32_t ntiles = p.ctile[p.chunks];
  for (uint32_t v = blockIdx.x; v < ((ntiles + (8u << a.run_bits) - 1u) & ~((8u << a.run_bits) - 1u)); v += gridDim.x) {
    const uint32_t t = xcd_tile(v, a.run_bits);
    if (t >= ntiles) { continue; }
    for (uint32_t b = threadIdx.x; b < bins; b += THREADS) { hist[b] = 0u; }
    PartTile tile{0u, 0u, 0ull};
    const auto count_one = [&](unsigned long long r) {
      if (r != kRecAbsent) { atomicAdd(&hist[(((uint32_t)(r >> 32) - a.bias) >> a.shift) & (bins - 1u)], 1u); }
    };
    if constexpr (SPAN) {
      (void)part_span<TILE / THREADS, THREADS>(p, a.tile, t, span, [&](uint32_t, uint64_t place) { count_one(p.in[place]); });
    } else {
      tile = part_tile(p, a.tile, t, sh);
#pragma unroll
      for (uint32_t k = 0; k < TILE / THREADS; ++k) {
        const uint32_t j = k * THREADS + threadIdx.x;
        if (j < tile.count) { count_one(p.in[tile.first + j]); }
      }
    }
    __syncthreads();
    for (uint32_t b = threadIdx.x; b < bins; b += THREADS) { p.cnt[part_flat(a, p, tile.c, t, b)] = hist[b]; }
    __syncthreads();
  }
}

constexpr uint32_t kFlatChunk = 4096;
constexpr uint32_t kFlatPer = kFlatChunk / 256u;
struct FlatScanArgs { uint32_t * v[kMaxIdx]; const uint32_t * units[kMaxIdx]; uint32_t unit_bits; uint64_t fixed[kMaxIdx]; uint32_t * partial[kMaxIdx]; uint32_t * total[kMaxIdx]; };
__device__ __forceinline__ uint64_t flat_length(const FlatScanArgs & a, uint32_t i) {
  return a.units[i] != nullptr ? ((uint64_t)*a.units[i] << a.unit_bits) + 1u : a.fixed[i];
}

__global__ __launch_bounds__(256) void k_flat_sums(const FlatScanArgs a) {
  __shared__ uint64_t smem[4];
  const uint32_t * v = a.v[blockIdx.y];
  const uint64_t m = flat_length(a, blockIdx.y);
  for (uint64_t blk = blockIdx.x; blk * kFlatChunk < m; blk += gridDim.x) {
    const uint64_t base = blk * kFlatChunk + (uint64_t)threadIdx.x * kFlatPer;
    uint64_t s = 0;
#pragma unroll
    for (uint32_t k = 0; k < kFlatPer; ++k) { if (base + k < m) { s += v[base + k]; } }
    uint64_t total;
    (void)block_exclusive_scan(s, smem, total);
    if (threadIdx.x == 0) { a.partial[blockIdx.y][blk] = (uint32_t)total; }
  }
}

__global__ __launch_bounds__(256) void k_flat_apply(const FlatScanArgs a) {
  __shared__ uint64_t smem[4];
  uint32_t * v = a.v[blockIdx.y];
  const uint64_t m = flat_length(a, blockIdx.y);
  const uint32_t * partial = a.partial[blockIdx.y];
  const uint64_t nblk = (m + kFlatChunk - 1) / kFlatChunk;
  for (uint64_t blk = blockIdx.x; blk < nblk; blk += gridDim.x) {
    uint64_t before = 0;
    for (uint64_t q = threadIdx.x; q < blk; q += 256u) { before += partial[q]; }
    uint64_t prefix;
    (void)block_exclusive_scan(before, smem, prefix);
    const uint64_t base = blk * kFlatChunk + (uint64_t)threadIdx.x * kFlatPer;
    uint32_t c[kFlatPer];
    uint64_t s = 0;
#pragma unroll
    for (uint32_t k = 0; k < kFlatPer; ++k) { c[k] = base + k < m ? v[base + k] : 0u; s += c[k]; }
    uint64_t total;
    uint64_t run = prefix + block_exclusive_scan(s, smem, total);
#pragma unroll
    for (uint32_t k = 0; k < kFlatPer; ++k) { if (base + k < m) { v[base + k] = (uint32_t)run; } run += c[k]; }
    if (blk + 1 == nblk && threadIdx.x == 0) { *a.total[blockIdx.y] = (uint32_t)(prefix + total); }
  }
}

template <uint32_t THREADS>
__device__ __forceinline__ uint64_t block_exclusive_scan_of(uint64_t v, uint64_t * smem, uint64_t & total) {
  const uint32_t lane = threadIdx.x & 63u, wave = threadIdx.x >> 6;
  uint64_t incl = v;
#pragma unroll
  for (unsigned d = 1; d < 64; d <<= 1) { const uint64_t t = swa_shfl_up_u64(incl, d); if (lane >= d) { incl += t; } }
  if (lane == 63u) { smem[wave] = incl; }
  __syncthreads();
  uint64_t wave_off = 0, tot = 0;
#pragma unroll
  for (uint32_t w = 0; w < THREADS / 64u; ++w) { const uint64_t x = smem[w]; wave_off += w < wave ? x : 0ull; tot += x; }
  __syncthreads();
  total = tot;
  return wave_off + incl - v;
}

template <int MODE, uint32_t TILE, uint32_t BINS, uint32_t THREADS, bool SPAN = false>
__global__ __launch_bounds__(THREADS) __attribute__((amdgpu_waves_per_eu(SPAN && THREADS == 512 ? 8 : 1))) void k_part_scatter(const PartArgs a) {
  constexpr uint32_t kPartPer = TILE / THREADS;
  extern __shared__ __attribute__((aligned(16))) unsigned long long part_lds[];
  unsigned long long * stage = part_lds;
  uint32_t * hist = reinterpret_cast<uint32_t *>(stage + TILE);
  uint32_t * lstart = hist + BINS;
  uint32_t * goff = lstart + BINS;
  __shared__ uint64_t smem[THREADS / 64u];
  __shared__ uint32_t sh[1];
  __shared__ typename std::conditional<SPAN, SpanLds, uint32_t>::type span;
  const PartIdx & p = a.p[blockIdx.y];
  const uint32_t bins = 1u << a.bits;
  const uint32_t ntiles = p.ctile[p.chunks];
  for (uint32_t v = blockIdx.x; v < ((ntiles + (8u << a.run_bits) - 1u) & ~((8u << a.run_bits) - 1u)); v += gridDim.x) {
    const uint32_t t = xcd_tile(v, a.run_bits);
    if (t >= ntiles) { continue; }
    for (uint32_t b = threadIdx.x; b < bins; b += THREADS) { hist[b] = 0u; }
    PartTile tile{0u, 0u, 0ull};
    unsigned long long rec[kPartPer];
    uint32_t pos[kPartPer];
    const auto digit_of = [&](unsigned long long r) { return (((uint32_t)(r >> 32) - a.bias) >> a.shift) & (bins - 1u); };
    if constexpr (SPAN) {
#pragma unroll
      for (uint32_t k = 0; k < kPartPer; ++k) { rec[k] = kRecAbsent; pos[k] = 0u; }
      (void)part_span<kPartPer, THREADS>(p, TILE, t, span, [&](uint32_t k, uint64_t place) {
        rec[k] = p.in[place];
        if (rec[k] != kRecAbsent) { pos[k] = atomicAdd(&hist[digit_of(rec[k])], 1u); }
      });
    } else {
      tile = part_tile(p, TILE, t, sh);
#pragma unroll
      for (uint32_t k = 0; k < kPartPer; ++k) {
        const uint32_t j = k * THREADS + threadIdx.x;
        rec[k] = kRecAbsent; pos[k] = 0u;
        if (j < tile.count) { rec[k] = p.in[tile.first + j]; }
        if (rec[k] != kRecAbsent) { pos[k] = atomicAdd(&hist[digit_of(rec[k])], 1u); }
      }
    }
    __syncthreads();
    {
      constexpr uint32_t kB = (BINS + THREADS - 1u) / THREADS;
      uint32_t h[kB];
      uint64_t sum = 0;
#pragma unroll
      for (uint32_t q = 0; q < kB; ++q) { const uint32_t b = kB * threadIdx.x + q; h[q] = b < bins ? hist[b] : 0u; sum += h[q]; }
      uint64_t total;
      uint32_t run = (uint32_t)block_exclusive_scan_of<THREADS>(sum, smem, total);
#pragma unroll
      for (uint32_t q = 0; q < kB; ++q) {
        const uint32_t b = kB * threadIdx.x + q;
        if (b < bins) { lstart[b] = run; goff[b] = p.cnt[part_flat(a, p, tile.c, t, b)]; }
        run += h[q];
      }
    }
    __syncthreads();
#pragma unroll
    for (uint32_t k = 0; k < kPartPer; ++k) {
      if (rec[k] != kRecAbsent) {
        const uint32_t at = lstart[(((uint32_t)(rec[k] >> 32) - a.bias) >> a.shift) & (bins - 1u)] + pos[k];
        stage[at] = rec[k];
      }
    }
    __syncthreads();
    const uint32_t present = lstart[bins - 1u] + hist[bins - 1u];
#pragma unroll
    for (uint32_t k = 0; k < kPartPer; ++k) {
      const uint32_t j = k * THREADS + threadIdx.x;
      if (j < present) {
        const unsigned long long r = stage[j];
        const uint32_t d = (((uint32_t)(r >> 32) - a.bias) >> a.shift) & (bins - 1u);
        const uint64_t g = (uint64_t)goff[d] + (j - lstart[d]);
        if (g < p.out_cap) {
          if (MODE == 2) { p.out32[g] = (uint32_t)r; } else { p.out[g] = r; }
        }
      }
    }
    __syncthreads();
  }
}

constexpr size_t part_scatter_lds(uint32_t tile, uint32_t bins) { return (size_t)tile * 8u + 3u * (size_t)bins * 4u; }

__global__ __launch_bounds__(256) void k_part_starts(const PartArgs a) {
  const PartIdx & p = a.p[blockIdx.y];
  const uint32_t segs = a.single_seg != 0u ? 1u : p.chunks;
  const uint64_t buckets = (uint64_t)segs << a.bits;
  for (uint64_t i = (uint64_t)blockIdx.x * blockDim.x + threadIdx.x; i <= buckets; i += (uint64_t)gridDim.x * blockDim.x) {
    if (i == buckets) { p.next_start[i] = *p.total; continue; }
    const uint32_t c = (uint32_t)(i >> a.bits), b = (uint32_t)i & ((1u << a.bits) - 1u);
    p.next_start[i] = p.cnt[a.single_seg != 0u ? (uint64_t)b * p.ctile[p.chunks] : ((uint64_t)p.ctile[c] << a.bits) + (uint64_t)b * (p.ctile[c + 1] - p.ctile[c])];
  }
}

struct GroupIdx {
  unsigned long long * rec;
  const uint64_t * bstart;
  uint32_t buckets;
  uint32_t * members;
  unsigned long long * items_tmp;
  uint32_t * kind_cnt;
};
struct GroupArgs {
  GroupIdx g[kMaxIdx];
  uint32_t pair_big, group_cap;
  uint32_t * flags;
  unsigned long long * guard;
  uint8_t * over;
};

constexpr uint32_t kG1Threads = 1024;
constexpr uint32_t kG1SlotBits = 13, kG1Slots = 1u << kG1SlotBits;
constexpr uint32_t kG1DupBits = 14, kG1DupSlots = 1u << kG1DupBits;
constexpr uint32_t kG1Target = 10240;
constexpr size_t kG1LdsBytes = kG1Slots * 4 * 2 + kG1DupSlots * 4;
static_assert(kG1Slots * 4 <= kG1DupSlots * 4, "the groups' places lie in the area behind the two tables");
constexpr uint32_t kG1OverBit = 0x80000000u;

constexpr uint32_t kG1Per = 8;
constexpr uint32_t kG1Tail = 2;

__device__ __forceinline__ uint32_t g1_size(uint32_t w) { return w & 0xFFFFu; }
__device__ __forceinline__ uint32_t g1_class(uint32_t w) {
  const uint32_t bits = (w >> 16) & 0x1Fu;
  return bits == 0u ? 0u : 31u - (uint32_t)__clz((int)bits);
}
__device__ __forceinline__ bool g1_over(uint32_t w, uint32_t cap) { return g1_size(w) > 1u && (g1_size(w) > cap || g1_class(w) >= kTooLong); }
__device__ __forceinline__ uint32_t g1_list(uint32_t w, uint32_t pair_big, uint32_t cap) {
  const uint32_t g = g1_size(w);
  if (g < 2u || g1_over(w, cap)) { return kListsPerIndex; }
  const uint32_t kind = g <= kSeedsPerItem ? pair_class(g) : (g <= pair_big ? kPairClasses : kPairClasses + 1u);
  return g1_class(w) * kListKinds + kind;
}
constexpr uint32_t kG1LineBits = kG1SlotBits - 2u, kG1Lines = 1u << kG1LineBits;
__device__ __forceinline__ uint32_t g1_home_line(uint32_t kk) { return (kk * 0x9E3779B1u) >> (32u - kG1LineBits); }

__device__ __forceinline__ uint32_t g1_enter(uint32_t * tcnt, uint32_t idx, uint32_t cls) {
  const uint32_t old = atomicAdd(&tcnt[idx], 1u);
  if (cls != 0u && (old >> (16u + cls) & 1u) == 0u) { atomicOr(&tcnt[idx], 1u << (16u + cls)); }
  return (old & 0xFFFFu) << kG1SlotBits | idx;
}
__device__ __forceinline__ uint32_t g1_find4(const uint4 & q, uint32_t v) {
  return q.x == v ? 0u : q.y == v ? 1u : q.z == v ? 2u : q.w == v ? 3u : 4u;
}

template <uint32_t N>
__device__ __forceinline__ bool g1_count_keys(uint32_t * tkey, uint32_t * tcnt, const uint32_t (&key)[N], uint32_t valid, uint32_t (&sr)[N]) {
  uint32_t line[N];
#pragma unroll
  for (uint32_t k = 0; k < N; ++k) { line[k] = g1_home_line(key[k] & ~7u); sr[k] = 0u; }
  uint32_t pend = valid;
  for (uint32_t rounds = 0; pend != 0u; ++rounds) {
    if (rounds > kG1Slots + kG1Lines) { return false; }
    uint4 q[N];
#pragma unroll
    for (uint32_t k = 0; k < N; ++k) { if ((pend >> k & 1u) != 0u) { q[k] = *reinterpret_cast<const uint4 *>(tkey + 4u * line[k]); } }
    uint32_t at[N];
#pragma unroll
    for (uint32_t k = 0; k < N; ++k) {
      at[k] = 4u;
      if ((pend >> k & 1u) == 0u) { continue; }
      const uint32_t want = (key[k] & ~7u) | 1u;
      at[k] = g1_find4(q[k], want);
      if (at[k] == 4u) {
        const uint32_t e = g1_find4(q[k], 0u);
        if (e == 4u) {
          line[k] = (line[k] + 1u) & (kG1Lines - 1u);
        } else {
          const uint32_t old = atomicCAS(&tkey[4u * line[k] + e], 0u, want);
          if (old == 0u || old == want) { at[k] = e; }
        }
      }
    }
#pragma unroll
    for (uint32_t k = 0; k < N; ++k) {
      if ((pend >> k & 1u) != 0u && at[k] < 4u) { sr[k] = g1_enter(tcnt, 4u * line[k] + at[k], key[k] & 7u); pend &= ~(1u << k); }
    }
  }
  return true;
}

constexpr uint32_t kG1Staged = kG1Slots + (kG1DupSlots - kG1Slots);
template <bool STAGED>
__device__ __forceinline__ void g1_place(const GroupArgs & a, const GroupIdx & g, const uint32_t * toff, uint32_t * staged, uint64_t start, uint32_t id, uint32_t sr, uint32_t which) {
  const uint32_t t = toff[sr & (kG1Slots - 1u)];
  const uint32_t at = (t & ~kG1OverBit) + (sr >> kG1SlotBits);
  if (STAGED) { staged[at] = id; } else { g.members[start + at] = id; }
  if ((t & kG1OverBit) != 0u) { atomicOr(reinterpret_cast<unsigned int *>(a.over + (id & ~3u)), (1u << which) << (8u * (id & 3u))); }
}

__device__ __forceinline__ uint32_t lanes_below(unsigned long long mask) {
  return __builtin_amdgcn_mbcnt_hi((uint32_t)(mask >> 32), __builtin_amdgcn_mbcnt_lo((uint32_t)mask, 0u));
}

__device__ __forceinline__ bool g1_count_once(uint32_t * tkey, uint32_t * tcnt, uint32_t key, uint32_t & sr) {
  const uint32_t want = (key & ~7u) | 1u, first = 4u * g1_home_line(key & ~7u);
  const uint4 q = *reinterpret_cast<const uint4 *>(tkey + first);
  uint32_t at = g1_find4(q, want);
  if (at == 4u) {
    const uint32_t e = g1_find4(q, 0u);
    if (e < 4u) {
      const uint32_t old = atomicCAS(&tkey[first + e], 0u, want);
      if (old == 0u || old == want) { at = e; }
    }
  }
  if (at == 4u) { return false; }
  sr = g1_enter(tcnt, first + at, key & 7u);
  return true;
}
__device__ __forceinline__ unsigned long long block_exclusive_scan64_1024(unsigned long long v, unsigned long long * smem16, unsigned long long & total, uint32_t tid) {
  const uint32_t lane = tid & 63u, wave = tid >> 6;
  unsigned long long incl = v;
#pragma unroll
  for (int d = 1; d < 64; d <<= 1) {
    const unsigned long long up = (unsigned long long)(uint32_t)__shfl_up((int)(uint32_t)incl, (unsigned)d, 64)
                                | (unsigned long long)(uint32_t)__shfl_up((int)(uint32_t)(incl >> 32), (unsigned)d, 64) << 32;
    if ((int)lane >= d) { incl += up; }
  }
  if (lane == 63u) { smem16[wave] = incl; }
  __syncthreads();
  unsigned long long x = lane < 16u ? smem16[lane] : 0ull;
#pragma unroll
  for (int d = 1; d < 16; d <<= 1) {
    const unsigned long long up = (unsigned long long)(uint32_t)__shfl_up((int)(uint32_t)x, (unsigned)d, 64)
                                | (unsigned long long)(uint32_t)__shfl_up((int)(uint32_t)(x >> 32), (unsigned)d, 64) << 32;
    if ((int)lane >= d) { x += up; }
  }
// ... 158 lines not shown
        } else if (lane == (uint32_t)(__ffsll((long long)same) - 1)) {
          atomicAdd(&kcnt[l], (uint32_t)__popcll(same));
        }
        todo &= ~same;
      }
    }
    __syncthreads();
    if (tid < 64u) {
      const uint32_t mine = tid < kListsPerIndex ? kcnt[tid] : 0u;
      uint32_t incl = mine;
#pragma unroll
      for (int d = 1; d < 32; d <<= 1) { const uint32_t up = (uint32_t)__shfl_up((int)incl, (unsigned)d, 64); if ((int)lane >= d) { incl += up; } }
      if (tid < kListsPerIndex) { kbase[tid] = incl - mine; g.kind_cnt[tid * g.buckets + b] = mine; kcnt[tid] = 0u; }
    }
    if (tid >= 64u && tid < 67u) {
      const uint32_t j = tid - 64u;
      const uint32_t sum = j == 0u ? gsum[0] - gsum[1] - gsum[2] : gsum[j];
      if (sum != 0u) { atomicAdd(a.guard + 2u + 2u * j + which, (unsigned long long)sum); }
    }
    __syncthreads();
    if (tid == 64u) { gsum[2] = 0u; }
    for (uint32_t i0 = 0; i0 < n_listed; i0 += kG1Threads) {
      const uint32_t i = i0 + tid;
      const uint32_t sl = i < n_listed ? glist[i] : 0u;
      const uint32_t w = i < n_listed ? tcnt[sl] : 0u;
      const uint32_t sz = g1_size(w);
      const uint32_t list = i < n_listed ? g1_list(w, a.pair_big, cap) : kListsPerIndex;
      const unsigned long long item = (unsigned long long)(uint32_t)(start + (toff[sl] & ~kG1OverBit)) | ((unsigned long long)sz << 32);
      unsigned long long todo = __ballot(list < kListsPerIndex);
      while (todo != 0ull) {
        const uint32_t l = lane_value(list, __ffsll((long long)todo) - 1);
        const unsigned long long same = __ballot(list == l);
        if (l % kListKinds == kPairClasses + 1u) {
          if (list == l) {
            const uint32_t tiles = (sz + kSeedsPerItem - 1u) / kSeedsPerItem;
            uint32_t at = kbase[l] + atomicAdd(&kcnt[l], tiled_item_count(sz));
            for (uint32_t r2 = 0; r2 < tiles; ++r2) {
              const uint32_t parts = (tiles - r2 + kTiledCols - 1u) / kTiledCols;
              for (uint32_t q = 0; q < parts; ++q) { g.items_tmp[start + at++] = item | ((unsigned long long)(r2 | (q << 6)) << 48); }
            }
          }
        } else {
          const int first = __ffsll((long long)same) - 1;
          uint32_t at = 0;
          if ((int)lane == first) { at = atomicAdd(&kcnt[l], (uint32_t)__popcll(same)); }
          at = lane_value(at, first);
          if (list == l) { g.items_tmp[start + kbase[l] + at + lanes_below(same)] = item; }
        }
        todo &= ~same;
      }
    }
    auto place_all = [&](auto staged_c) {
      constexpr bool STAGED = decltype(staged_c)::value;
      unsigned long long trec[kG1Tail];
#pragma unroll
      for (uint32_t t = 0; t < kG1Tail; ++t) {
        const uint32_t r = (kG1Per + t) * kG1Threads + tid;
        trec[t] = (here >> (kG1Per + t) & 1u) != 0u ? g.rec[start + r] : 0ull;
      }
#pragma unroll
      for (uint32_t k = 0; k < kG1Per; ++k) {
        if ((here >> k & 1u) != 0u) { g1_place<STAGED>(a, g, toff, staged, start, rid[k], rkey[k], which); }
      }
#pragma unroll
      for (uint32_t t = 0; t < kG1Tail; ++t) {
        if ((here >> (kG1Per + t) & 1u) != 0u) { g1_place<STAGED>(a, g, toff, staged, start, (uint32_t)trec[t], (uint32_t)(trec[t] >> 32), which); }
      }
      for (uint32_t r = (kG1Per + kG1Tail) * kG1Threads + tid; r < c; r += kG1Threads) {
        const unsigned long long rec = g.rec[start + r];
        g1_place<STAGED>(a, g, toff, staged, start, (uint32_t)rec, (uint32_t)(rec >> 32), which);
      }
    };
    if (c <= kG1Staged) {
      __syncthreads();
      place_all(std::true_type{});
      __syncthreads();
      for (uint32_t i = tid; i < c; i += kG1Threads) { g.members[start + i] = staged[i]; }
    } else {
      place_all(std::false_type{});
    }
    __syncthreads();
  }
}

struct ListIdx {
  const unsigned long long * items_tmp;
  const uint64_t * bstart;
  const uint32_t * kind_pos;
  uint32_t buckets;
  PairLists l;
};
struct ListArgs { ListIdx x[kMaxIdx]; };

__global__ __launch_bounds__(256) void k_group_lists(const ListArgs a) {
  const ListIdx & x = a.x[blockIdx.y];
  const uint32_t lane = threadIdx.x & 63u;
  const uint32_t nwaves = gridDim.x * 4u;
  const uint64_t entries = (uint64_t)kListsPerIndex * x.buckets;
  for (uint32_t b = blockIdx.x * 4u + (threadIdx.x >> 6); b < x.buckets; b += nwaves) {
    const uint64_t start = x.bstart[b];
    uint32_t my_pos = 0, my_cnt = 0, my_first = 0;
    if (lane < kListsPerIndex) {
      const uint64_t e = (uint64_t)lane * x.buckets + b;
      my_pos = x.kind_pos[e]; my_cnt = x.kind_pos[e + 1] - my_pos;
      my_first = x.kind_pos[(uint64_t)lane * x.buckets];
    }
    uint32_t local = 0;
    unsigned long long todo = __ballot(my_cnt != 0u);
    while (todo != 0ull) {
      const int l = __ffsll((long long)todo) - 1;
      todo &= todo - 1ull;
      const uint32_t cnt = lane_value(my_cnt, l), at = lane_value(my_pos, l) - lane_value(my_first, l);
      const uint64_t base = x.l.region.at[(uint32_t)l / kListKinds][(uint32_t)l % kListKinds];
      const uint64_t room = x.l.region.at[(uint32_t)l / kListKinds][(uint32_t)l % kListKinds + 1u] - base;
      for (uint32_t j = lane; j < cnt; j += 64u) {
        const unsigned long long it = x.items_tmp[start + local + j];
        swa_item item;
        item.begin = (uint32_t)it; item.size = (uint32_t)(it >> 32) & 0xFFFFu; item.chunk = (uint32_t)(it >> 48);
        if ((uint64_t)at + j < room) { x.l.items[base + at + j] = item; }
      }
      local += cnt;
    }
  }
  if (blockIdx.x == 0 && threadIdx.x < kListsPerIndex) {
    const uint32_t l = threadIdx.x;
    const uint32_t len = x.kind_pos[l + 1u < kListsPerIndex ? (uint64_t)(l + 1u) * x.buckets : entries] - x.kind_pos[(uint64_t)l * x.buckets];
    const uint64_t room = x.l.region.at[l / kListKinds][l % kListKinds + 1u] - x.l.region.at[l / kListKinds][l % kListKinds];
    x.l.counters[(l / kListKinds) * 8u + l % kListKinds] = (uint32_t)min((uint64_t)len, room);
  }
}

__global__ __launch_bounds__(256) void k_stream_fallback(const uint32_t * __restrict__ seqlen, uint32_t first, uint32_t count,
                                                         const uint8_t * __restrict__ over, swa_fallback * list, uint32_t * list_counter,
                                                         uint32_t owner_rank, uint32_t owner_world, const uint64_t * __restrict__ seqs,
                                                         const uint64_t * __restrict__ seq_off, uint32_t minlen) {
  for (uint32_t k = blockIdx.x * blockDim.x + threadIdx.x; k < count; k += gridDim.x * blockDim.x) {
    const uint32_t seed = first + k;
    const bool plain = seqlen[seed] < minlen;
    if (plain) {
      if (owner_world == 1u || seed % owner_world == owner_rank) { list[atomicAdd(list_counter, 1u)] = swa_fallback{seed, 0u}; }
      continue;
    }
    const uint32_t bits = over[seed];
    if ((bits & 1u) != 0u) { list[atomicAdd(list_counter, 1u)] = swa_fallback{seed, 1u}; }
    if ((bits & 2u) != 0u) { list[atomicAdd(list_counter, 1u)] = swa_fallback{seed, 2u}; }
  }
}

constexpr uint32_t kCsrMaxR = 9;
constexpr uint32_t kCsrStage = 1024;
constexpr uint32_t kCsrBigStage = 8192;
struct CsrArgs {
  const unsigned long long * links;
  const uint64_t * bstart;
  uint32_t buckets, r, first, count;
  uint64_t * offsets;
  uint32_t * neighbours;
  uint64_t cap;
  uint32_t * heavy;
  uint32_t * heavy_count;
  uint64_t * end_copy;
};

__device__ __forceinline__ void wave_sort_lds(uint32_t * v, uint32_t len, uint32_t lane) {
  for (uint32_t phase = 0; phase < len; ++phase) {
    for (uint32_t i = (phase & 1u) + 2u * lane; i + 1u < len; i += 128u) {
      const uint32_t x = v[i], y = v[i + 1u];
      if (x > y) { v[i] = y; v[i + 1u] = x; }
    }
    wave_lds_sync();
  }
}

__device__ __forceinline__ void sort_short_rows(uint32_t * stage, const uint32_t * off, uint32_t rows, uint32_t first_row, uint32_t step) {
  for (uint32_t i = first_row; i < rows; i += step) {
    const uint32_t lo = off[i], hi = off[i + 1u];
    if (hi - lo > 32u) { continue; }
    for (uint32_t x = lo + 1u; x < hi; ++x) {
      const uint32_t v = stage[x];
      uint32_t y = x;
      while (y > lo && stage[y - 1u] > v) { stage[y] = stage[y - 1u]; --y; }
      stage[y] = v;
    }
  }
}

__device__ __forceinline__ void order2(uint32_t & x, uint32_t & y) { const uint32_t lo = min(x, y), hi = max(x, y); x = lo; y = hi; }
template <int N>
__device__ __forceinline__ void sort_row_in_registers(uint32_t * row, uint32_t len) {
  uint32_t v[N];
#pragma unroll
  for (int k = 0; k < N; ++k) { v[k] = (uint32_t)k < len ? row[k] : 0xFFFFFFFFu; }
#pragma unroll
  for (int k = 2; k <= N; k <<= 1) {
#pragma unroll
    for (int j = k >> 1; j > 0; j >>= 1) {
#pragma unroll
      for (int i = 0; i < N; ++i) {
        const int l = i ^ j;
        if (l > i) { if ((i & k) == 0) { order2(v[i], v[l]); } else { order2(v[l], v[i]); } }
      }
    }
  }
#pragma unroll
  for (int k = 0; k < N; ++k) { if ((uint32_t)k < len) { row[k] = v[k]; } }
}
__device__ __forceinline__ void wave_rank_sort64(uint32_t * row, uint32_t len, uint32_t lane) {
  const bool have = lane < len;
  const uint32_t mine = have ? row[lane] : 0xFFFFFFFFu;
  uint32_t rank = 0;
  for (uint32_t y = 0; y < len; ++y) { const uint32_t u = row[y]; rank += (u < mine || (u == mine && y < lane)) ? 1u : 0u; }
  wave_lds_sync();
  if (have) { row[rank] = mine; }
  wave_lds_sync();
}
template <uint32_t ROWS_MAX>
__device__ __forceinline__ void sort_rows_of_wave(uint32_t * stage, const uint32_t * off, uint32_t rows, uint32_t lane) {
  uint32_t lo[ROWS_MAX / 64u], len[ROWS_MAX / 64u];
#pragma unroll
  for (uint32_t q = 0; q < ROWS_MAX / 64u; ++q) {
    const uint32_t i = lane + 64u * q;
    lo[q] = i < rows ? off[i] : 0u; len[q] = i < rows ? off[i + 1u] - lo[q] : 0u;
    if (len[q] >= 2u && len[q] <= 4u) { sort_row_in_registers<4>(stage + lo[q], len[q]); }
    if (len[q] > 4u && len[q] <= 8u) { sort_row_in_registers<8>(stage + lo[q], len[q]); }
    if (len[q] > 8u && len[q] <= 16u) { sort_row_in_registers<16>(stage + lo[q], len[q]); }
  }
#pragma unroll
  for (uint32_t q = 0; q < ROWS_MAX / 64u; ++q) {
    unsigned long long todo = __ballot(len[q] > 16u);
    while (todo != 0ull) {
      const int src = __ffsll((long long)todo) - 1;
      todo &= todo - 1ull;
      const uint32_t l = lane_value(len[q], src), at = lane_value(lo[q], src);
      if (l <= 64u) { wave_rank_sort64(stage + at, l, lane); } else { wave_sort_lds(stage + at, l, lane); }
    }
  }
}

template <int RB>
__global__ __launch_bounds__(256) void k_csr_bucket(const CsrArgs a) {
  __shared__ uint32_t cnt_all[4][1u << RB];
  __shared__ uint32_t off_all[4][(1u << RB) + 1u];
  __shared__ uint32_t stage_all[4][kCsrStage];
  const uint32_t wave = threadIdx.x >> 6, lane = threadIdx.x & 63u;
  uint32_t * cnt = cnt_all[wave];
  uint32_t * off = off_all[wave];
  uint32_t * stage = stage_all[wave];
  const uint32_t rows = 1u << a.r;
  const uint32_t nwaves = gridDim.x * 4u;
  for (uint32_t b = blockIdx.x * 4u + wave; b < a.buckets; b += nwaves) {
    const uint64_t start = a.bstart[b];
    const uint32_t c = (uint32_t)(a.bstart[b + 1] - start);
    const uint32_t row0 = b << a.r;
    if (c > kCsrStage) {
      if (lane == 0u) { a.heavy[atomicAdd(a.heavy_count, 1u)] = b; }
      continue;
    }
    for (uint32_t i = lane; i < rows; i += 64u) { cnt[i] = 0u; }
    wave_lds_sync();
    constexpr uint32_t kPer = kCsrStage / 64u;
    const uint32_t turns = (c + 63u) >> 6;
    uint32_t dst[kPer], rowpos[kPer];
#pragma unroll
    for (uint32_t k = 0; k < kPer; ++k) {
      if (k >= turns) { break; }
      const uint32_t j = k * 64u + lane;
      const unsigned long long e = j < c ? a.links[start + j] : 0ull;
      dst[k] = (uint32_t)e;
      rowpos[k] = ((uint32_t)(e >> 32) - a.first) & (rows - 1u);
    }
#pragma unroll
    for (uint32_t k = 0; k < kPer; ++k) {
      if (k >= turns) { break; }
      if (k * 64u + lane < c) { rowpos[k] |= atomicAdd(&cnt[rowpos[k]], 1u) << 16; }
    }
    wave_lds_sync();
    {
      const uint32_t per = (rows + 63u) >> 6;
      uint32_t s = 0;
      for (uint32_t k = 0; k < per; ++k) { const uint32_t i = lane * per + k; s += i < rows ? cnt[i] : 0u; }
      uint32_t incl = s;
#pragma unroll
      for (int d = 1; d < 64; d <<= 1) { const uint32_t up = (uint32_t)__shfl_up((int)incl, (unsigned)d, 64); if ((int)lane >= d) { incl += up; } }
      uint32_t run = incl - s;
      for (uint32_t k = 0; k < per; ++k) { const uint32_t i = lane * per + k; if (i < rows) { off[i] = run; run += cnt[i]; } }
      if (lane == 63u) { off[rows] = run; }
    }
    wave_lds_sync();
    for (uint32_t i = lane; i < rows; i += 64u) { if (row0 + i < a.count) { a.offsets[row0 + i] = start + off[i]; } }
    if (b + 1u == a.buckets && lane == 0u) { a.offsets[a.count] = start + c; *a.end_copy = start + c; }
#pragma unroll
    for (uint32_t k = 0; k < kPer; ++k) {
      if (k >= turns) { break; }
      if (k * 64u + lane < c) { stage[off[rowpos[k] & 0xFFFFu] + (rowpos[k] >> 16)] = dst[k]; }
    }
    wave_lds_sync();
    sort_rows_of_wave<(1u << RB)>(stage, off, rows, lane);
    wave_lds_sync();
#pragma unroll
    for (uint32_t k = 0; k < kPer; ++k) {
      if (k >= turns) { break; }
      const uint32_t j = k * 64u + lane;
      if (j < c && start + j < a.cap) { a.neighbours[start + j] = stage[j]; }
    }
    wave_lds_sync();
  }
}

__global__ __launch_bounds__(256) void k_csr_bucket_big(const CsrArgs a) {
  __shared__ uint32_t cnt[1u << kCsrMaxR];
  __shared__ uint32_t off[(1u << kCsrMaxR) + 1u];
  __shared__ uint32_t stage[kCsrBigStage];
  __shared__ uint64_t smem[4];
  const uint32_t wave = threadIdx.x >> 6, lane = threadIdx.x & 63u;
  const uint32_t rows = 1u << a.r;
  const uint32_t nheavy = *a.heavy_count;
  for (uint32_t h = blockIdx.x; h < nheavy; h += gridDim.x) {
    const uint32_t b = a.heavy[h];
    const uint64_t start = a.bstart[b];
    const uint32_t c = (uint32_t)(a.bstart[b + 1] - start);
    const uint32_t row0 = b << a.r;
    for (uint32_t i = threadIdx.x; i < rows; i += 256u) { cnt[i] = 0u; }
    __syncthreads();
    for (uint32_t j = threadIdx.x; j < c; j += 256u) { atomicAdd(&cnt[((uint32_t)(a.links[start + j] >> 32) - a.first) & (rows - 1u)], 1u); }
    __syncthreads();
    {
      const uint32_t i0 = 2u * threadIdx.x, i1 = i0 + 1u;
      const uint32_t c0 = i0 < rows ? cnt[i0] : 0u, c1 = i1 < rows ? cnt[i1] : 0u;
      uint64_t total;
      const uint32_t ex = (uint32_t)block_exclusive_scan((uint64_t)c0 + c1, smem, total);
      if (i0 < rows) { off[i0] = ex; }
      if (i1 < rows) { off[i1] = ex + c0; }
      if (threadIdx.x == 0) { off[rows] = (uint32_t)total; }
    }
    __syncthreads();
    for (uint32_t i = threadIdx.x; i < rows; i += 256u) {
      if (row0 + i < a.count) { a.offsets[row0 + i] = start + off[i]; }
      cnt[i] = off[i];
    }
    if (b + 1u == a.buckets && threadIdx.x == 0) { a.offsets[a.count] = start + c; *a.end_copy = start + c; }
    __syncthreads();
    if (c <= kCsrBigStage) {
      for (uint32_t j = threadIdx.x; j < c; j += 256u) {
        const unsigned long long e = a.links[start + j];
        stage[atomicAdd(&cnt[((uint32_t)(e >> 32) - a.first) & (rows - 1u)], 1u)] = (uint32_t)e;
      }
      __syncthreads();
      sort_short_rows(stage, off, rows, threadIdx.x, 256u);
      for (uint32_t i = wave; i < rows; i += 4u) {
        const uint32_t lo = off[i], len = off[i + 1u] - lo;
        if (len > 32u) { wave_sort_lds(stage + lo, len, lane); }
      }
      __syncthreads();
      for (uint32_t j = threadIdx.x; j < c; j += 256u) { if (start + j < a.cap) { a.neighbours[start + j] = stage[j]; } }
    } else if (start + c <= a.cap) {
      for (uint32_t j = threadIdx.x; j < c; j += 256u) {
        const unsigned long long e = a.links[start + j];
        a.neighbours[start + atomicAdd(&cnt[((uint32_t)(e >> 32) - a.first) & (rows - 1u)], 1u)] = (uint32_t)e;
      }
      __threadfence();
      __syncthreads();
      uint32_t * mine = stage + wave * (kCsrBigStage / 4u);
      for (uint32_t i = wave; i < rows; i += 4u) {
        const uint32_t lo = off[i], len = off[i + 1u] - lo;
        if (len < 2u) { continue; }
        uint32_t * row = a.neighbours + start + lo;
        if (len <= kCsrBigStage / 4u) {
          for (uint32_t x = lane; x < len; x += 64u) { mine[x] = row[x]; }
          wave_lds_sync();
          wave_sort_lds(mine, len, lane);
          for (uint32_t x = lane; x < len; x += 64u) { row[x] = mine[x]; }
          wave_lds_sync();
        } else {
          for (uint32_t phase = 0; phase < len; ++phase) {
            for (uint32_t x = (phase & 1u) + 2u * lane; x + 1u < len; x += 128u) {
              const uint32_t u = row[x], v = row[x + 1u];
              if (u > v) { row[x] = v; row[x + 1u] = u; }
            }
            __threadfence_block();
            __builtin_amdgcn_wave_barrier();
          }
        }
      }
    }
    __syncthreads();
  }
}
```

swarm_amd/csrc/swa_internal.h:

```cpp
#pragma once

#include <hip/hip_runtime.h>

#include <cstdint>
#include <cstdio>
#include <cstdlib>
#include <cstring>
#include <string>
#include <vector>

#include "../../include/swarm_amd.h"

struct alignas(16) swa_slot {
  uint64_t hash;
  uint32_t amp;
  uint32_t pad;
};

struct swa_dbuf {
  void * ptr = nullptr;
  size_t bytes = 0;
};

struct swa_ctx {
  int device = 0;
  hipStream_t stream = nullptr;
  bool own_stream = false;
  int num_cus = 256;
  std::string err;

  bool timing = false;
  hipEvent_t ev[32] = {};
  bool ev_ready = false;
  bool ev_used[16] = {};

  swa_db_view db{};
  bool db_owned = false;
  swa_dbuf d_seqs, d_seq_off, d_seqlen, d_abund;

  bool d1_ready = false;
  uint64_t table_size = 0;
  uint64_t bloom_words = 0;
  uint32_t zobrist_len = 0;
  uint32_t zobrist_resident = 0;
  bool patterns_resident = false;
  swa_dbuf d_zobrist, d_seqhash, d_table, d_bloom, d_patterns;
  swa_dbuf d_status;
  void * h_status = nullptr;
  swa_dbuf d_flags;
  swa_dbuf d_stats;
  swa_dbuf d_edges;
  swa_dbuf d_counts, d_cursor, d_scan_tmp, d_offsets_tmp, d_nb_tmp;
  bool anchor_usable = false;
  bool anchor_ready = false;
  bool full_index = false;
  const uint32_t * route_ids[2] = {nullptr, nullptr};
  const unsigned long long * route_rec[2] = {nullptr, nullptr};
  uint32_t route_m[2] = {0, 0};
  bool rank_ready = false;
  bool db_unordered = false;
  bool props_ready = false;
  uint32_t db_shortest = 0;
  uint32_t class_pop[8] = {};
  bool windows_ready = false;
  uint32_t windows_chosen = 0;
  uint32_t owner_rank = 0, owner_world = 1;
  uint32_t anchor_a = 0, anchor_b = 0;
  uint32_t anchor_w = 32;
  uint32_t windows_w = 32;
  swa_dbuf d_guard;
  bool guard_index = false;
  bool guard_keys_done = false;
  bool guard_keys_pending = false;
  swa_dbuf d_aux, d_akeys[1], d_acounts[1], d_aitems[2];
  swa_dbuf d_acounters, d_afallback, d_arank, d_rank_tmp;
  swa_dbuf d_seg_fill;
  swa_dbuf d_seg_base;
  uint64_t seg_cap = 0;

  bool qgram_ready = false;
  swa_dbuf d_qgrams, d_list_a, d_list_b, d_list_c, d_list_d;
  uint64_t pen_mismatch = 18, pen_gapopen = 24, pen_gapextend = 13, resolution = 1;
  bool search_ready = false;
  uint32_t wfa_steps = 0;
  uint32_t wfa_ring = 0;
  swa_dbuf d_wfa;

  bool scan_ready = false;
  swa_dbuf d_scan_est, d_scan_swarmed, d_scan_targets, d_scan_diffs, d_scan_hits, d_scan_counters;
  swa_dbuf d_scan_cand;
  swa_dbuf d_scan_seeds;
  swa_dbuf d_scan_compares;
  uint32_t scan_cand_bound = 0;
  void * h_scan_pinned = nullptr;
  std::vector<uint32_t> scan_host, scan_perm, scan_idx_tmp;
  std::vector<uint64_t> scan_sorted;
  uint64_t scan_pair_cap = 0;
  uint64_t scan_launches = 0;

  swa_dbuf d_light, d_graft, d_bloomflex, d_fpatterns, d_queue, d_fcounters;
  swa_dbuf d_frole, d_fkeys, d_fcnt, d_foff, d_fslot, d_fmembers, d_fitems, d_fpairs;
  uint64_t fast_pair_cap = 0;

  uint32_t dn_shortest = 0;
  bool dn_graph_ready = false, dn_graph_ncb = false;
  uint64_t dn_pair_cap = 0, dn_comparisons = 0, dn_aligned = 0, dn_launches = 0, dn_edges = 0, dn_work = 0;
  swa_dbuf d_dn_keys, d_dn_vals;
  uint32_t dn_owner_rank = 0, dn_owner_world = 1;

  bool lines_ready = false;
  uint32_t lines_quads = 0;
  uint32_t list_counts[2 * 4 * 8] = {};
  bool list_counts_ready = false;
  uint64_t list_regions_items = 0;
  bool stream_index = false;
  uint32_t stream_extra_bits = 0;
  swa_dbuf d_stream[30];
  bool member_index = false, only_oversized = false;
  uint32_t over_mass = 0;
  uint64_t mtable_size = 0, mbloom_words = 0;

  bool csr_ready = false;
  uint32_t index_first = 0, index_count = 0;
  bool index_routed = false;
  uint32_t guard_retries = 0;
  swa_dbuf d_words_stage;
  const void * staged_first = nullptr; uint64_t staged_words = 0;
  bool cluster_ready = false;
  uint32_t cluster_maxgen = 0;
  int pair_blocks[4] = {};
  bool g1_lds_opt_in = false;
  bool part_lds_opt_in = false;
  uint32_t pair_lds_opt_in = 0;
  bool csr_has_diffs = false;
  uint64_t csr_total = 0;
  swa_dbuf d_cluster, d_cluster_ctl;

  std::vector<uint32_t> nw_seqlen;
  uint64_t nw_totals[4] = {};
  swa_dbuf d_nw_ids, d_nw_lists, d_nw_res, d_nw_text, d_nw_gather;
};

int swa_fail(swa_ctx * ctx, int code, const char * what, hipError_t e);
int swa_fail_msg(swa_ctx * ctx, int code, const std::string & msg);
inline void swa_lap(swa_ctx * ctx, const char * what);
int swa_reserve(swa_ctx * ctx, swa_dbuf & buf, size_t bytes);
void swa_release(swa_dbuf & buf);
int swa_hash_sequences(swa_ctx * ctx);
int swa_dn_graph_compute(swa_ctx * ctx, int no_cluster_breaking);
int swa_dn_graph_emit(swa_ctx * ctx, const unsigned long long * sorted, const uint32_t * svals, uint64_t nedges, uint64_t * offsets,
                      uint32_t * neighbours, uint8_t * diffs, uint64_t cap, uint64_t * total);

int swa_d1_csr_from_lists(swa_ctx * ctx, const unsigned long long * d_links, const uint64_t * starts, const uint64_t * counts, uint32_t lists,
                          uint64_t * d_offsets, uint32_t * d_neighbours, uint64_t cap);

inline void swa_t0(swa_ctx * ctx, int slot) {
  if (ctx->timing && ctx->ev_ready) { (void)hipEventRecord(ctx->ev[2 * slot], ctx->stream); }
}
inline void swa_t1(swa_ctx * ctx, int slot) {
  if (ctx->timing && ctx->ev_ready) { (void)hipEventRecord(ctx->ev[2 * slot + 1], ctx->stream); ctx->ev_used[slot] = true; }
}

#define SWA_HIP(ctx, expr)                                                     \
  do {                                                                         \
    hipError_t e_ = (expr);                                                    \
    if (e_ != hipSuccess) return swa_fail((ctx), SWA_E_DEVICE, #expr, e_);     \
  } while (0)

#define SWA_TRY(expr)                  \
  do {                                 \
    int rc_ = (expr);                  \
    if (rc_ != SWA_OK) return rc_;     \
  } while (0)

void swa_zobrist_table(uint32_t zobrist_len, std::vector<uint64_t> & tab);
void swa_bloom_patterns(uint32_t count, uint32_t k, std::vector<uint64_t> & pat);
uint64_t swa_hashtable_size(uint64_t n);

#ifdef __HIPCC__

__device__ __forceinline__ unsigned swa_nt(const uint64_t * seq, uint32_t pos) {
  return (unsigned)((seq[pos >> 5] >> ((pos & 31u) << 1)) & 3u);
}

__device__ __forceinline__ uint64_t swa_shfl_u64(uint64_t v, int src) {
  const int lo = __shfl((int)(uint32_t)v, src, 64);
  const int hi = __shfl((int)(uint32_t)(v >> 32), src, 64);
  return ((uint64_t)(uint32_t)hi << 32) | (uint32_t)lo;
}
__device__ __forceinline__ uint64_t swa_shfl_xor_u64(uint64_t v, int mask) {
  const int lo = __shfl_xor((int)(uint32_t)v, mask, 64);
  const int hi = __shfl_xor((int)(uint32_t)(v >> 32), mask, 64);
  return ((uint64_t)(uint32_t)hi << 32) | (uint32_t)lo;
}
__device__ __forceinline__ uint64_t swa_shfl_up_u64(uint64_t v, unsigned d) {
  const int lo = __shfl_up((int)(uint32_t)v, d, 64);
  const int hi = __shfl_up((int)(uint32_t)(v >> 32), d, 64);
  return ((uint64_t)(uint32_t)hi << 32) | (uint32_t)lo;
}
__device__ __forceinline__ uint64_t swa_shfl_down_u64(uint64_t v, unsigned d) {
  const int lo = __shfl_down((int)(uint32_t)v, d, 64);
  const int hi = __shfl_down((int)(uint32_t)(v >> 32), d, 64);
  return ((uint64_t)(uint32_t)hi << 32) | (uint32_t)lo;
}

__device__ __forceinline__ uint64_t swa_variant_word(const uint64_t * seed, uint32_t nw, uint32_t type,
                                                     uint32_t pos, uint32_t base, uint32_t w) {
  const uint32_t wp = pos >> 5;
  const uint32_t sh = (pos & 31u) << 1;
  const uint64_t cur = (w < nw) ? seed[w] : 0ull;
  if (type == 0u) {
    if (w != wp) return cur;
    return (cur & ~(3ull << sh)) | ((uint64_t)base << sh);
  }
  const uint64_t lowmask = (1ull << sh) - 1ull;
  if (type == 1u) {
    const uint64_t nxt = (w + 1 < nw) ? seed[w + 1] : 0ull;
    const uint64_t shifted = (cur >> 2) | (nxt << 62);
    if (w < wp) return cur;
    if (w > wp) return shifted;
    return (cur & lowmask) | (shifted & ~lowmask);
  }
  {
    const uint64_t prv = (w >= 1 && w - 1 < nw) ? seed[w - 1] : 0ull;
    const uint64_t shifted = (cur << 2) | (prv >> 62);
    if (w < wp) return cur;
    if (w > wp) return shifted;
    return (cur & lowmask) | ((uint64_t)base << sh) | (shifted & ~(lowmask | (3ull << sh)));
  }
}

#endif

#include "host/pool.h"
inline void swa_touch_pages(void * ptr, size_t bytes) {
  if (ptr == nullptr || bytes < (size_t(4) << 20)) { return; }
  char * p = static_cast<char *>(ptr);
  const size_t pages = (bytes + 4095) / 4096;
  const unsigned parts = std::min<unsigned>(swa_pool::get().size(), 16u);
  swa_pool::get().run(parts, [&](unsigned t) {
    for (size_t k = pages * t / parts; k < pages * (t + 1) / parts; ++k) {
      p[k * 4096] = 0;
    }
  });
}

#include <chrono>
inline void swa_lap(swa_ctx * ctx, const char * what) {
  static const bool on = std::getenv("SWARM_AMD_STEP_TIMING") != nullptr;
  if (!on) { return; }
  static auto last = std::chrono::steady_clock::now();
  (void)hipStreamSynchronize(ctx->stream);
  const auto now = std::chrono::steady_clock::now();
  std::fprintf(stderr, "[step] %-34s %8.3f ms\n", what, 1e3 * std::chrono::duration<double>(now - last).count());
  last = std::chrono::steady_clock::now();
}
```

Measured before the change: 6.037 billion amplicons/s.

## Fuse flat scan into single-pass decoupled-lookback kernel and pack CSR links to 32 bits

Replaces the two-launch flat scan (sums plus apply) and the separate k_part_starts launch with one chained scan kernel. It uses decoupled lookback over epoch-tagged granules and falls back to a recompute when a block gives up spinning. Separately, the CSR build can now have the final partition pass emit 32-bit packed (row,target) links instead of 64-bit ones, which halves link traffic in the CSR bucket kernels. The cost is extra scratch buffers, a spin-wait that depends on forward progress, and an environment-variable fallback path.

After: 5.987 billion amplicons/s (median of 3 runs). About the same (-0.8%).

```diff
diff --git a/swarm_amd/csrc/d1.hip b/swarm_amd/csrc/d1.hip
--- a/swarm_amd/csrc/d1.hip
+++ b/swarm_amd/csrc/d1.hip
@@ -767,7 +767,9 @@
 __global__ void k_set_guard_made(unsigned long long * guard, uint32_t made0, uint32_t made1) { guard[0] = made0; guard[1] = made1; }
 
 enum { kSbLines = 0, kSbRec = 1, kSbFp = 5, kSbCnt = 8, kSbTile = 10, kSbStart = 12, kSbPartial = 14, kSbScal = 16,
-       kSbMembers = 17, kSbOver = 19, kSbKind = 20, kSbLinkA = 22, kSbLinkB = 23, kSbHeavy = 24, kSbMTable = 26, kSbMBloom = 27, kSbSched = 28 };
+       kSbMembers = 17, kSbOver = 19, kSbKind = 20, kSbLinkA = 22, kSbLinkB = 23, kSbHeavy = 24, kSbMTable = 26, kSbMBloom = 27, kSbSched = 28,
+       kSbOff = 30, kSbChain = 32 };
+constexpr uint32_t kChainGaveUpWord = 120;
 
 struct PartPlan { uint32_t levels; uint32_t bits[4]; uint32_t total; };
 static PartPlan plan_levels(uint32_t total_bits, uint32_t max_bits = kPartMaxBits) {
@@ -794,6 +796,7 @@
   bool hist0_done = false;
   PartPlan plan{};
   uint32_t * out32[kMaxIdx] = {};
+  uint32_t * off[kMaxIdx] = {};
   uint32_t * cnt[kMaxIdx] = {}; uint32_t * ctile[kMaxIdx] = {}; uint64_t * starts[kMaxIdx] = {}; uint32_t * partial[kMaxIdx] = {};
   uint32_t * total[kMaxIdx] = {};
   uint64_t starts_stride = 0;
@@ -831,6 +834,84 @@
   if (c.n == 0 || most == 0) { return SWA_OK; }
   hipLaunchKernelGGL(k_clear_many, dim3(grid_for(ctx, most, 256, 8)), dim3(256), 0, ctx->stream, c);
   SWA_HIP(ctx, hipGetLastError());
+  return SWA_OK;
+}
+
+static int chain_state(swa_ctx * ctx, uint32_t i, uint64_t chunks, unsigned long long ** granule, uint32_t ** tickets) {
+  swa_dbuf & b = ctx->d_stream[kSbChain + i];
+  const void * had = b.ptr;
+  const size_t had_bytes = b.bytes;
+  SWA_TRY(swa_reserve(ctx, b, (chunks + 8) * sizeof(uint64_t)));
+  if (b.ptr != had || b.bytes != had_bytes) { SWA_HIP(ctx, hipMemsetAsync(b.ptr, 0, b.bytes, ctx->stream)); }
+  *tickets = static_cast<uint32_t *>(b.ptr);
+  *granule = static_cast<unsigned long long *>(b.ptr) + 8;
+  return SWA_OK;
+}
+
+static int scan_flat(swa_ctx * ctx, const FlatScanArgs & f, uint32_t nidx, uint64_t max_len, const PartArgs * part, uint64_t buckets) {
+  const uint64_t cu_grid = (uint64_t)ctx->num_cus * 8;
+  const uint64_t nblk = std::max<uint64_t>((max_len + kFlatChunk - 1) / kFlatChunk, 1);
+  const dim3 grid((unsigned)std::min<uint64_t>(nblk, cu_grid), nidx);
+  if (ctx->chain_scan_off || getenv("SWA_SCAN_TWO_LAUNCH") != nullptr) {
+    hipLaunchKernelGGL(k_flat_sums, grid, dim3(256), 0, ctx->stream, f);
+    hipLaunchKernelGGL(k_flat_apply, grid, dim3(256), 0, ctx->stream, f);
+    if (part != nullptr) {
+      PartArgs a = *part;
+      for (uint32_t i = 0; i < nidx; ++i) { a.p[i].cnt = f.out[i]; }
+      hipLaunchKernelGGL(k_part_starts, dim3((unsigned)std::min<uint64_t>((buckets + 256) / 256, cu_grid), nidx), dim3(256), 0, ctx->stream, a);
+    }
+    SWA_HIP(ctx, hipGetLastError());
+    return SWA_OK;
+  }
+  if (++ctx->chain_epoch >= (1u << 30)) {
+    for (uint32_t i = 0; i < kMaxIdx; ++i) {
+      swa_dbuf & b = ctx->d_stream[kSbChain + i];
+      if (b.ptr != nullptr) { SWA_HIP(ctx, hipMemsetAsync(b.ptr, 0, b.bytes, ctx->stream)); }
+    }
+    ctx->chain_epoch = 1;
+  }
+  ChainArgs c{};
+  c.unit_bits = f.unit_bits;
+  c.single_seg = part != nullptr ? part->single_seg : 0u;
+  c.epoch = ctx->chain_epoch;
+  c.gave_up = static_cast<uint32_t *>(ctx->d_status.ptr) + kChainGaveUpWord;
+  for (uint32_t i = 0; i < nidx; ++i) {
+    ChainIdx & x = c.x[i];
+    x.v = f.v[i]; x.out = f.out[i]; x.units = f.units[i]; x.fixed = f.fixed[i]; x.total = f.total[i];
+    uint32_t * tickets = nullptr;
+    SWA_TRY(chain_state(ctx, i, nblk, &x.granule, &tickets));
+    if (i == 0) { c.tickets = tickets; }
+    if (part != nullptr) { x.next_start = part->p[i].next_start; x.ctile = part->p[i].ctile; x.chunks = part->p[i].chunks; }
+  }
+  hipLaunchKernelGGL(k_chain_scan, dim3((unsigned)std::min<uint64_t>(nblk, (uint64_t)ctx->num_cus), nidx), dim3(256), 0, ctx->stream, c);
+  SWA_HIP(ctx, hipGetLastError());
+  return SWA_OK;
+}
+static void chain_note_status(swa_ctx * ctx, const uint32_t * status_u32) {
+  if (status_u32[kChainGaveUpWord] != 0u) { ctx->chain_scan_off = true; }
+}
+
+extern "C" int swa_test_flat_scan(swa_ctx * ctx, const uint32_t * d_v, uint64_t len, const uint32_t * d_ctile, uint32_t chunks, uint32_t bits,
+                                  int single, uint32_t * d_out, uint64_t * d_next_start, uint32_t * d_total, int two_launch, uint32_t * gave_up) {
+  SWA_HIP(ctx, hipSetDevice(ctx->device));
+  FlatScanArgs f{};
+  f.v[0] = d_v; f.out[0] = d_out; f.total[0] = d_total;
+  f.unit_bits = d_ctile != nullptr ? bits : 0u;
+  f.units[0] = d_ctile != nullptr ? d_ctile + chunks : nullptr;
+  f.fixed[0] = len;
+  SWA_TRY(swa_reserve(ctx, ctx->d_stream[kSbPartial], (len / kFlatChunk + 2) * sizeof(uint32_t)));
+  f.partial[0] = static_cast<uint32_t *>(ctx->d_stream[kSbPartial].ptr);
+  PartArgs a{};
+  a.single_seg = single ? 1u : 0u; a.bits = bits;
+  a.p[0].ctile = const_cast<uint32_t *>(d_ctile); a.p[0].chunks = chunks; a.p[0].next_start = d_next_start; a.p[0].total = d_total;
+  const uint64_t buckets = (uint64_t)(single ? 1u : chunks) << bits;
+  const bool was_off = ctx->chain_scan_off;
+  ctx->chain_scan_off = two_launch != 0;
+  const int rc = scan_flat(ctx, f, 1, len, d_ctile != nullptr ? &a : nullptr, buckets);
+  ctx->chain_scan_off = was_off;
+  SWA_TRY(rc);
+  SWA_HIP(ctx, hipMemcpyAsync(gave_up, static_cast<uint32_t *>(ctx->d_status.ptr) + kChainGaveUpWord, sizeof(uint32_t), hipMemcpyDeviceToHost, ctx->stream));
+  SWA_HIP(ctx, hipStreamSynchronize(ctx->stream));
   return SWA_OK;
 }
 
@@ -876,12 +957,12 @@
     else if (wide) { hipLaunchKernelGGL((k_part_hist<1024, kPartTileMax, 256>), grid_t, dim3(256), 0, ctx->stream, a); }
     else if (a.span != 0u) { hipLaunchKernelGGL((k_part_hist<512, kPartTileMax, 256, true>), grid_t, dim3(256), 0, ctx->stream, a); }
     else { hipLaunchKernelGGL((k_part_hist<512, kPartTileMax, 256>), grid_t, dim3(256), 0, ctx->stream, a); }
+    const uint64_t next_chunks = (single ? 1 : chunks) << bits;
     FlatScanArgs f{};
     f.unit_bits = bits;
-    for (uint32_t i = 0; i < j.nidx; ++i) { f.v[i] = j.cnt[i]; f.units[i] = j.ctile[i] + chunks; f.partial[i] = j.partial[i]; f.total[i] = j.total[i]; }
-    const dim3 grid_f((unsigned)std::min<uint64_t>(((tiles << bits) + 1 + kFlatChunk - 1) / kFlatChunk, (uint64_t)cu_grid), j.nidx);
-    hipLaunchKernelGGL(k_flat_sums, grid_f, dim3(256), 0, ctx->stream, f);
-    hipLaunchKernelGGL(k_flat_apply, grid_f, dim3(256), 0, ctx->stream, f);
+    for (uint32_t i = 0; i < j.nidx; ++i) { f.v[i] = j.cnt[i]; f.out[i] = j.off[i]; f.units[i] = j.ctile[i] + chunks; f.partial[i] = j.partial[i]; f.total[i] = j.total[i]; }
+    SWA_TRY(scan_flat(ctx, f, j.nidx, (tiles << bits) + 1, &a, next_chunks));
+    for (uint32_t i = 0; i < j.nidx; ++i) { a.p[i].cnt = j.off[i]; }
     if (wide && j.tile == 8192) {
       constexpr size_t lds = part_scatter_lds(8192, 1024);
       if (!ctx->part_lds_opt_in) {
@@ -892,13 +973,12 @@
     }
     else if (wide) { hipLaunchKernelGGL((k_part_scatter<0, 4096, 1024, 512>), grid_t, dim3(512), part_scatter_lds(4096, 1024), ctx->stream, a); }
     else if (j.tile == 2048) { hipLaunchKernelGGL((k_part_scatter<0, 2048, 512, 512>), grid_t, dim3(512), part_scatter_lds(2048, 512), ctx->stream, a); }
-    else if (a.span != 0u && low_halves) { hipLaunchKernelGGL((k_part_scatter<2, 4096, 512, 512, true>), grid_t, dim3(512), part_scatter_lds(4096, 512), ctx->stream, a); }
+    else if (a.span != 0u && low_halves) { hipLaunchKernelGGL((k_part_scatter<3, 4096, 512, 512, true>), grid_t, dim3(512), part_scatter_lds(4096, 512), ctx->stream, a); }
     else if (a.span != 0u) { hipLaunchKernelGGL((k_part_scatter<0, 4096, 512, 512, true>), grid_t, dim3(512), part_scatter_lds(4096, 512), ctx->stream, a); }
-    else if (low_halves) { hipLaunchKernelGGL((k_part_scatter<2, 4096, 512, 512>), grid_t, dim3(512), part_scatter_lds(4096, 512), ctx->stream, a); }
+    else if (low_halves) { hipLaunchKernelGGL((k_part_scatter<3, 4096, 512, 512>), grid_t, dim3(512), part_scatter_lds(4096, 512), ctx->stream, a); }
     else { hipLaunchKernelGGL((k_part_scatter<0, 4096, 512, 512>), grid_t, dim3(512), part_scatter_lds(4096, 512), ctx->stream, a); }
-    chunks = (single ? 1 : chunks) << bits;
+    chunks = next_chunks;
     single = false;
-    hipLaunchKernelGGL(k_part_starts, dim3((unsigned)std::min<uint64_t>((chunks + 256) / 256, (uint64_t)cu_grid), j.nidx), dim3(256), 0, ctx->stream, a);
     SWA_HIP(ctx, hipGetLastError());
   }
   j.buckets = (uint32_t)chunks;
@@ -967,6 +1047,7 @@
   for (int i = 0; i < 2; ++i) {
     for (int h = 0; h < 2; ++h) { SWA_TRY(swa_reserve(ctx, ctx->d_stream[kSbRec + 2 * i + h], (records + 1) * sizeof(uint64_t))); }
     SWA_TRY(swa_reserve(ctx, ctx->d_stream[kSbCnt + i], e_cnt * sizeof(uint32_t)));
+    SWA_TRY(swa_reserve(ctx, ctx->d_stream[kSbOff + i], std::max<uint64_t>(e_cnt, (uint64_t)kListsPerIndex * buckets + 2) * sizeof(uint32_t)));
     SWA_TRY(swa_reserve(ctx, ctx->d_stream[kSbTile + i], e_tile * sizeof(uint32_t)));
     SWA_TRY(swa_reserve(ctx, ctx->d_stream[kSbStart + i], (2 * e_start + 4) * sizeof(uint64_t)));
     SWA_TRY(swa_reserve(ctx, ctx->d_stream[kSbPartial + i], e_partial * sizeof(uint32_t)));
@@ -1042,6 +1123,7 @@
     j.in[i] = by_rec ? ctx->route_rec[i] : j.buf[i][1];
     j.cstart0[i] = nullptr; j.cstride0[i] = routed ? ctx->route_m[i] : n;
     j.cnt[i] = static_cast<uint32_t *>(ctx->d_stream[kSbCnt + i].ptr);
+    j.off[i] = static_cast<uint32_t *>(ctx->d_stream[kSbOff + i].ptr);
     j.ctile[i] = static_cast<uint32_t *>(ctx->d_stream[kSbTile + i].ptr);
     j.starts[i] = static_cast<uint64_t *>(ctx->d_stream[kSbStart + i].ptr);
     j.partial[i] = static_cast<uint32_t *>(ctx->d_stream[kSbPartial + i].ptr);
@@ -1097,18 +1179,16 @@
   ListArgs la{};
   auto * acounters = static_cast<uint32_t *>(ctx->d_acounters.ptr);
   for (int i = 0; i < 2; ++i) {
-    f.v[i] = g.g[i].kind_cnt; f.units[i] = nullptr; f.fixed[i] = (uint64_t)kListsPerIndex * buckets + 1;
+    f.v[i] = g.g[i].kind_cnt; f.out[i] = j.off[i]; f.units[i] = nullptr; f.fixed[i] = (uint64_t)kListsPerIndex * buckets + 1;
     f.partial[i] = j.partial[i]; f.total[i] = reinterpret_cast<uint32_t *>(scal + 10 + i);
     ListIdx & x = la.x[i];
-    x.items_tmp = g.g[i].items_tmp; x.bstart = g.g[i].bstart; x.kind_pos = g.g[i].kind_cnt; x.buckets = (uint32_t)buckets;
+    x.items_tmp = g.g[i].items_tmp; x.bstart = g.g[i].bstart; x.kind_pos = j.off[i]; x.buckets = (uint32_t)buckets;
     x.l.items = static_cast<swa_item *>(ctx->d_aitems[i].ptr);
     x.l.region = regions;
     x.l.counters = acounters + kCounterBase + (uint32_t)i * kWidthClasses * 8u;
     x.l.pair_big = g.pair_big;
   }
-  const dim3 grid_k((unsigned)std::min<uint64_t>(((uint64_t)kListsPerIndex * buckets + kFlatChunk) / kFlatChunk, (uint64_t)ctx->num_cus * 8), 2);
-  hipLaunchKernelGGL(k_flat_sums, grid_k, dim3(256), 0, ctx->stream, f);
-  hipLaunchKernelGGL(k_flat_apply, grid_k, dim3(256), 0, ctx->stream, f);
+  SWA_TRY(scan_flat(ctx, f, 2, (uint64_t)kListsPerIndex * buckets + 1, nullptr, 0));
   hipLaunchKernelGGL(k_group_lists, dim3((unsigned)std::min<uint64_t>((buckets + 3) / 4, (uint64_t)ctx->num_cus * 8), 2), dim3(256), 0, ctx->stream, la);
   SWA_HIP(ctx, hipGetLastError());
   swa_lap(ctx, "groups + work lists");
@@ -1121,7 +1201,7 @@
 
 static int csr_from_chunks(swa_ctx * ctx, uint32_t first, uint32_t count, const unsigned long long * links, const uint64_t * d_cstart, uint64_t cstride,
                            const uint32_t * d_csize, uint32_t chunks, uint32_t csize_cap, uint64_t max_tiles0, uint64_t link_cap,
-                           uint64_t * d_offsets, uint32_t * d_neighbours, uint64_t cap) {
+                           uint64_t * d_offsets, uint32_t * d_neighbours, uint64_t cap, bool may_pack = false) {
   uint32_t nbits = 1;
   while (nbits < 32 && ((uint64_t)1 << nbits) < count) { ++nbits; }
   uint32_t r = std::min<uint32_t>(8, nbits - 1);
@@ -1140,6 +1220,7 @@
   SWA_TRY(swa_reserve(ctx, ctx->d_stream[kSbLinkA], (link_cap + 1) * sizeof(uint64_t)));
   SWA_TRY(swa_reserve(ctx, ctx->d_stream[kSbLinkB], (link_cap + 1) * sizeof(uint64_t)));
   SWA_TRY(swa_reserve(ctx, ctx->d_stream[kSbCnt], e_cnt * sizeof(uint32_t)));
+  SWA_TRY(swa_reserve(ctx, ctx->d_stream[kSbOff], e_cnt * sizeof(uint32_t)));
   SWA_TRY(swa_reserve(ctx, ctx->d_stream[kSbTile], e_tile * sizeof(uint32_t)));
   SWA_TRY(swa_reserve(ctx, ctx->d_stream[kSbStart], (2 * e_start + 4) * sizeof(uint64_t)));
   SWA_TRY(swa_reserve(ctx, ctx->d_stream[kSbPartial], e_partial * sizeof(uint32_t)));
@@ -1150,17 +1231,21 @@
   j.cstart0[0] = d_cstart; j.cstride0[0] = cstride;
   j.csize0[0] = d_csize;
   j.cnt[0] = static_cast<uint32_t *>(ctx->d_stream[kSbCnt].ptr);
+  j.off[0] = static_cast<uint32_t *>(ctx->d_stream[kSbOff].ptr);
   j.ctile[0] = static_cast<uint32_t *>(ctx->d_stream[kSbTile].ptr);
   j.starts[0] = static_cast<uint64_t *>(ctx->d_stream[kSbStart].ptr);
   j.partial[0] = static_cast<uint32_t *>(ctx->d_stream[kSbPartial].ptr);
   auto * extra = static_cast<uint64_t *>(ctx->d_status.ptr) + 48;
   j.total[0] = reinterpret_cast<uint32_t *>(extra + 1);
   j.starts_stride = e_start + 2;
+  const uint64_t target_bound = std::max<uint64_t>(ctx->db.n, (uint64_t)first + count);
+  const bool packed = may_pack && r >= 1 && target_bound <= (1ull << (32 - r)) && getenv("SWA_CSR_WIDE") == nullptr;
+  if (packed) { j.out32[0] = reinterpret_cast<uint32_t *>(j.buf[0][(j.plan.levels - 1) & 1u]); }
   swa_t0(ctx, 13);
   SWA_TRY(run_partition(ctx, j));
   swa_t1(ctx, 13);
   CsrArgs c{};
-  c.links = j.out[0]; c.bstart = j.bstart[0]; c.buckets = j.buckets; c.r = r; c.first = first; c.count = count;
+  c.links = j.out[0]; c.links32 = packed ? j.out32[0] : nullptr; c.bstart = j.bstart[0]; c.buckets = j.buckets; c.r = r; c.first = first; c.count = count;
   c.offsets = d_offsets; c.neighbours = d_neighbours; c.cap = d_neighbours != nullptr ? cap : 0;
   SWA_TRY(swa_reserve(ctx, ctx->d_stream[kSbHeavy], ((uint64_t)j.buckets + 2) * sizeof(uint32_t)));
   c.heavy = static_cast<uint32_t *>(ctx->d_stream[kSbHeavy].ptr) + 1;
@@ -1168,13 +1253,19 @@
   c.end_copy = extra;
   SWA_HIP(ctx, hipMemsetAsync(c.heavy_count, 0, sizeof(uint32_t), ctx->stream));
   swa_t0(ctx, 14);
-  static const int csr_per_cu[2] = {
-    [] { int nb = 0; return hipOccupancyMaxActiveBlocksPerMultiprocessor(&nb, k_csr_bucket<8>, 256, 0) == hipSuccess && nb > 0 ? nb : 4; }(),
-    [] { int nb = 0; return hipOccupancyMaxActiveBlocksPerMultiprocessor(&nb, k_csr_bucket<9>, 256, 0) == hipSuccess && nb > 0 ? nb : 4; }() };
-  const dim3 cgrid((unsigned)std::min<uint64_t>(((uint64_t)j.buckets + 3) / 4, (uint64_t)ctx->num_cus * (uint64_t)csr_per_cu[r <= 8 ? 0 : 1]));
-  if (r <= 8) { hipLaunchKernelGGL(k_csr_bucket<8>, cgrid, dim3(256), 0, ctx->stream, c); }
-  else { hipLaunchKernelGGL(k_csr_bucket<9>, cgrid, dim3(256), 0, ctx->stream, c); }
-  hipLaunchKernelGGL(k_csr_bucket_big, dim3((unsigned)ctx->num_cus * 4), dim3(256), 0, ctx->stream, c);
+  static const int csr_per_cu[4] = {
+    [] { int nb = 0; return hipOccupancyMaxActiveBlocksPerMultiprocessor(&nb, k_csr_bucket<8, false>, 256, 0) == hipSuccess && nb > 0 ? nb : 4; }(),
+    [] { int nb = 0; return hipOccupancyMaxActiveBlocksPerMultiprocessor(&nb, k_csr_bucket<9, false>, 256, 0) == hipSuccess && nb > 0 ? nb : 4; }(),
+    [] { int nb = 0; return hipOccupancyMaxActiveBlocksPerMultiprocessor(&nb, k_csr_bucket<8, true>, 256, 0) == hipSuccess && nb > 0 ? nb : 4; }(),
+    [] { int nb = 0; return hipOccupancyMaxActiveBlocksPerMultiprocessor(&nb, k_csr_bucket<9, true>, 256, 0) == hipSuccess && nb > 0 ? nb : 4; }() };
+  const int form = (r <= 8 ? 0 : 1) + (packed ? 2 : 0);
+  const dim3 cgrid((unsigned)std::min<uint64_t>(((uint64_t)j.buckets + 3) / 4, (uint64_t)ctx->num_cus * (uint64_t)csr_per_cu[form]));
+  if (form == 0) { hipLaunchKernelGGL((k_csr_bucket<8, false>), cgrid, dim3(256), 0, ctx->stream, c); }
+  else if (form == 1) { hipLaunchKernelGGL((k_csr_bucket<9, false>), cgrid, dim3(256), 0, ctx->stream, c); }
+  else if (form == 2) { hipLaunchKernelGGL((k_csr_bucket<8, true>), cgrid, dim3(256), 0, ctx->stream, c); }
+  else { hipLaunchKernelGGL((k_csr_bucket<9, true>), cgrid, dim3(256), 0, ctx->stream, c); }
+  if (packed) { hipLaunchKernelGGL(k_csr_bucket_big<true>, dim3((unsigned)ctx->num_cus * 4), dim3(256), 0, ctx->stream, c); }
+  else { hipLaunchKernelGGL(k_csr_bucket_big<false>, dim3((unsigned)ctx->num_cus * 4), dim3(256), 0, ctx->stream, c); }
   swa_t1(ctx, 14);
   SWA_HIP(ctx, hipGetLastError());
   return SWA_OK;
@@ -1185,7 +1276,7 @@
   const uint64_t tiles_per_seg = (ctx->seg_cap + 4096 - 1) / 4096;
   return csr_from_chunks(ctx, first, count, static_cast<const unsigned long long *>(ctx->d_edges.ptr), nullptr, ctx->seg_cap,
                          static_cast<const uint32_t *>(ctx->d_seg_fill.ptr), nseg, (uint32_t)std::min<uint64_t>(ctx->seg_cap, 0xFFFFFFFFu),
-                         (uint64_t)nseg * tiles_per_seg + 2, link_cap, d_offsets, d_neighbours, cap);
+                         (uint64_t)nseg * tiles_per_seg + 2, link_cap, d_offsets, d_neighbours, cap, true);
 }
 
 #define SWA_PAIR_CASE(KERNEL, P, WW, NN) \
@@ -1494,6 +1585,7 @@
   SWA_HIP(ctx, hipMemcpyAsync(status, ctx->d_status.ptr, 512 * sizeof(uint32_t), hipMemcpyDeviceToHost, ctx->stream));
   SWA_HIP(ctx, hipStreamSynchronize(ctx->stream));
   const uint32_t * flags = status;
+  chain_note_status(ctx, status);
   *dups = flags[0];
   memcpy(ctx->list_counts, status + 256 + kCounterBase, sizeof(ctx->list_counts));
   ctx->list_counts_ready = true;
@@ -1778,6 +1870,7 @@
     const uint32_t anchor_overflow = reinterpret_cast<const uint32_t *>(status)[2];
     const uint64_t csr_end = status[48];
     const uint32_t links_sorted = (uint32_t)status[49];
+    chain_note_status(ctx, reinterpret_cast<const uint32_t *>(status));
     const bool guarded = ctx->anchor_usable;
     n_edges = got[0];
     if (guarded && anchor_overflow != 0) {
diff --git a/swarm_amd/csrc/d1_stream.inc b/swarm_amd/csrc/d1_stream.inc
--- a/swarm_amd/csrc/d1_stream.inc
+++ b/swarm_amd/csrc/d1_stream.inc
@@ -461,7 +461,7 @@
 
 constexpr uint32_t kFlatChunk = 4096;
 constexpr uint32_t kFlatPer = kFlatChunk / 256u;
-struct FlatScanArgs { uint32_t * v[kMaxIdx]; const uint32_t * units[kMaxIdx]; uint32_t unit_bits; uint64_t fixed[kMaxIdx]; uint32_t * partial[kMaxIdx]; uint32_t * total[kMaxIdx]; };
+struct FlatScanArgs { const uint32_t * v[kMaxIdx]; uint32_t * out[kMaxIdx]; const uint32_t * units[kMaxIdx]; uint32_t unit_bits; uint64_t fixed[kMaxIdx]; uint32_t * partial[kMaxIdx]; uint32_t * total[kMaxIdx]; };
 __device__ __forceinline__ uint64_t flat_length(const FlatScanArgs & a, uint32_t i) {
   return a.units[i] != nullptr ? ((uint64_t)*a.units[i] << a.unit_bits) + 1u : a.fixed[i];
 }
@@ -483,7 +483,8 @@
 
 __global__ __launch_bounds__(256) void k_flat_apply(const FlatScanArgs a) {
   __shared__ uint64_t smem[4];
-  uint32_t * v = a.v[blockIdx.y];
+  const uint32_t * v = a.v[blockIdx.y];
+  uint32_t * out = a.out[blockIdx.y];
   const uint64_t m = flat_length(a, blockIdx.y);
   const uint32_t * partial = a.partial[blockIdx.y];
   const uint64_t nblk = (m + kFlatChunk - 1) / kFlatChunk;
@@ -500,8 +501,148 @@
     uint64_t total;
     uint64_t run = prefix + block_exclusive_scan(s, smem, total);
 #pragma unroll
-    for (uint32_t k = 0; k < kFlatPer; ++k) { if (base + k < m) { v[base + k] = (uint32_t)run; } run += c[k]; }
+    for (uint32_t k = 0; k < kFlatPer; ++k) { if (base + k < m) { out[base + k] = (uint32_t)run; } run += c[k]; }
     if (blk + 1 == nblk && threadIdx.x == 0) { *a.total[blockIdx.y] = (uint32_t)(prefix + total); }
+  }
+}
+
+constexpr uint32_t kChainSpin = 1u << 20;
+constexpr uint32_t kChainLook = 4;
+struct ChainIdx {
+  const uint32_t * v;
+  uint32_t * out;
+  const uint32_t * units;
+  uint64_t fixed;
+  uint32_t * total;
+  unsigned long long * granule;
+  uint64_t * next_start;
+  const uint32_t * ctile;
+  uint32_t chunks;
+};
+struct ChainArgs { ChainIdx x[kMaxIdx]; uint32_t * tickets; uint32_t unit_bits; uint32_t single_seg; uint32_t epoch; uint32_t * gave_up; };
+
+__device__ __forceinline__ uint64_t chain_pos(const ChainIdx & x, const ChainArgs & a, uint64_t i) {
+  if (a.single_seg != 0u) { return i * x.ctile[x.chunks]; }
+  const uint32_t c = (uint32_t)(i >> a.unit_bits), b = (uint32_t)i & ((1u << a.unit_bits) - 1u);
+  const uint64_t t0 = x.ctile[c];
+  return (t0 << a.unit_bits) + (c < x.chunks ? (uint64_t)b * (x.ctile[c + 1u] - x.ctile[c]) : 0ull);
+}
+__device__ __forceinline__ uint32_t chain_first_at(const ChainIdx & x, const ChainArgs & a, uint32_t nb, uint64_t e, uint32_t lane) {
+  uint32_t lo = 0, hi = nb;
+  while (lo < hi) {
+    const uint32_t step = (hi - lo + 63u) >> 6;
+    const uint64_t i = (uint64_t)lo + (uint64_t)lane * step;
+    const bool ge = i >= hi || chain_pos(x, a, i) >= e;
+    const unsigned long long mk = __ballot(ge);
+    const uint32_t k = mk == 0ull ? 64u : (uint32_t)__ffsll((long long)mk) - 1u;
+    if (k == 0u) { break; }
+    const uint64_t up = (uint64_t)lo + (uint64_t)k * step;
+    lo = lo + (k - 1u) * step + 1u;
+    hi = (uint32_t)min(up, (uint64_t)hi);
+  }
+  return lo;
+}
+
+typedef __attribute__((address_space(1))) unsigned long long chain_g64;
+__device__ __forceinline__ void chain_publish(unsigned long long * g, uint32_t epoch, uint32_t state, uint32_t value) {
+  __hip_atomic_store((chain_g64 *)g, ((unsigned long long)epoch << 34) | ((unsigned long long)state << 32) | value, __ATOMIC_RELAXED, __HIP_MEMORY_SCOPE_AGENT);
+}
+
+__global__ __launch_bounds__(256) void k_chain_scan(const ChainArgs a) {
+  __shared__ uint32_t sval[kFlatChunk];
+  __shared__ uint64_t smem[4];
+  __shared__ uint32_t sh[6];
+  const ChainIdx & x = a.x[blockIdx.y];
+  const uint32_t lane = threadIdx.x & 63u, wave = threadIdx.x >> 6;
+  const uint64_t m = x.units != nullptr ? ((uint64_t)*x.units << a.unit_bits) + 1u : x.fixed;
+  const uint64_t nblk = (m + kFlatChunk - 1u) / kFlatChunk;
+  const uint32_t nb = x.next_start != nullptr ? ((a.single_seg != 0u ? 1u : x.chunks) << a.unit_bits) + 1u : 0u;
+  const uint32_t epoch = a.epoch & 0x3FFFFFFFu;
+  uint32_t * ticket = a.tickets + (epoch & 1u) * kMaxIdx + blockIdx.y;
+  if (blockIdx.x == 0 && blockIdx.y == 0 && threadIdx.x < kMaxIdx) { a.tickets[((epoch + 1u) & 1u) * kMaxIdx + threadIdx.x] = 0u; }
+  for (;;) {
+    if (threadIdx.x == 0) { sh[0] = atomicAdd(ticket, 1u); }
+    __syncthreads();
+    const uint32_t blk = sh[0];
+    if (blk >= nblk) { break; }
+    const uint64_t e0 = (uint64_t)blk * kFlatChunk, base = e0 + (uint64_t)threadIdx.x * kFlatPer;
+    uint32_t c[kFlatPer];
+    uint32_t s = 0;
+#pragma unroll
+    for (uint32_t k = 0; k < kFlatPer; ++k) { c[k] = base + k < m ? x.v[base + k] : 0u; s += c[k]; }
+    uint64_t agg64;
+    uint32_t run = (uint32_t)block_exclusive_scan((uint64_t)s, smem, agg64);
+    const uint32_t agg = (uint32_t)agg64;
+    if (wave == 0u) {
+      uint32_t prefix = 0, gave_up = 0;
+      if (blk == 0u) {
+        if (lane == 0u) { chain_publish(x.granule, epoch, 2u, agg); }
+      } else {
+        if (lane == 0u) { chain_publish(x.granule + blk, epoch, 1u, agg); }
+        int64_t at = (int64_t)blk - 1;
+        for (uint32_t spins = 0;;) {
+          unsigned long long g[kChainLook];
+#pragma unroll
+          for (uint32_t q = 0; q < kChainLook; ++q) {
+            const int64_t i = at - (int64_t)lane - 64 * (int64_t)q;
+            g[q] = i >= 0 ? __hip_atomic_load((chain_g64 *)(x.granule + i), __ATOMIC_RELAXED, __HIP_MEMORY_SCOPE_AGENT)
+                          : (((unsigned long long)epoch << 34) | (2ull << 32));
+          }
+          uint32_t p = 64u * kChainLook;
+          bool ok = true;
+          uint32_t mine = 0;
+#pragma unroll
+          for (uint32_t q = 0; q < kChainLook; ++q) {
+            const uint32_t st = (uint32_t)(g[q] >> 34) == epoch ? (uint32_t)(g[q] >> 32) & 3u : 0u;
+            const unsigned long long incl = __ballot(st == 2u), ready = __ballot(st != 0u);
+            if (p == 64u * kChainLook && incl != 0ull) { p = 64u * q + (uint32_t)__ffsll((long long)incl) - 1u; }
+            const unsigned long long need = p >= 64u * q + 63u ? ~0ull : (p < 64u * q ? 0ull : (2ull << (p - 64u * q)) - 1ull);
+            ok = ok && (ready & need) == need;
+            mine += ((need >> lane) & 1ull) != 0ull ? (uint32_t)g[q] : 0u;
+          }
+          if (ok) {
+#pragma unroll
+            for (int o = 32; o > 0; o >>= 1) { mine += (uint32_t)__shfl_xor((int)mine, o, 64); }
+            prefix += mine;
+            if (p < 64u * kChainLook) { break; }
+            at -= 64 * (int64_t)kChainLook;
+            continue;
+          }
+          if (++spins >= kChainSpin) { gave_up = 1u; break; }
+          __builtin_amdgcn_s_sleep(1);
+        }
+      }
+      if (lane == 0u) { sh[1] = prefix; sh[2] = gave_up; }
+    } else if (wave <= 2u && nb != 0u) {
+      const uint64_t e = wave == 1u ? e0 : min(e0 + kFlatChunk, m);
+      const uint32_t first = chain_first_at(x, a, nb, e, lane);
+      if (lane == 0u) { sh[2 + wave] = first; }
+    }
+    __syncthreads();
+    uint32_t prefix = sh[1];
+    if (sh[2] != 0u) {
+      uint64_t sum = 0;
+      for (uint64_t q = threadIdx.x; q < e0; q += 256u) { sum += x.v[q]; }
+      uint64_t all;
+      (void)block_exclusive_scan(sum, smem, all);
+      prefix = (uint32_t)all;
+      if (threadIdx.x == 0) { atomicAdd(a.gave_up, 1u); }
+    }
+    if (threadIdx.x == 0 && blk != 0u) { chain_publish(x.granule + blk, epoch, 2u, prefix + agg); }
+    run += prefix;
+#pragma unroll
+    for (uint32_t k = 0; k < kFlatPer; ++k) {
+      if (base + k < m) { x.out[base + k] = run; }
+      sval[threadIdx.x * kFlatPer + k] = run;
+      run += c[k];
+    }
+    if (blk + 1u == nblk && threadIdx.x == 0) { *x.total = prefix + agg; }
+    if (nb != 0u) {
+      __syncthreads();
+      const uint32_t i0 = sh[3], i1 = sh[4];
+      for (uint32_t i = i0 + threadIdx.x; i < i1; i += 256u) { x.next_start[i] = sval[chain_pos(x, a, i) - e0]; }
+    }
+    __syncthreads();
   }
 }
 
@@ -594,7 +735,8 @@
         const uint32_t d = (((uint32_t)(r >> 32) - a.bias) >> a.shift) & (bins - 1u);
         const uint64_t g = (uint64_t)goff[d] + (j - lstart[d]);
         if (g < p.out_cap) {
-          if (MODE == 2) { p.out32[g] = (uint32_t)r; } else { p.out[g] = r; }
+          if (MODE == 3) { p.out32[g] = (((uint32_t)(r >> 32) - a.bias) << (32u - a.shift)) | (uint32_t)r; }
+          else { p.out[g] = r; }
         }
       }
     }
@@ -1059,6 +1201,7 @@
 constexpr uint32_t kCsrBigStage = 8192;
 struct CsrArgs {
   const unsigned long long * links;
+  const uint32_t * links32;
   const uint64_t * bstart;
   uint32_t buckets, r, first, count;
   uint64_t * offsets;
@@ -1069,6 +1212,17 @@
   uint64_t * end_copy;
 };
 
+template <bool P32>
+__device__ __forceinline__ void csr_link(const CsrArgs & a, uint64_t j, uint32_t rows, uint32_t & row, uint32_t & target) {
+  if constexpr (P32) {
+    const uint32_t e = a.links32[j];
+    row = e >> (32u - a.r); target = e & (0xFFFFFFFFu >> a.r);
+  } else {
+    const unsigned long long e = a.links[j];
+    row = ((uint32_t)(e >> 32) - a.first) & (rows - 1u); target = (uint32_t)e;
+  }
+}
+
 __device__ __forceinline__ void wave_sort_lds(uint32_t * v, uint32_t len, uint32_t lane) {
   for (uint32_t phase = 0; phase < len; ++phase) {
     for (uint32_t i = (phase & 1u) + 2u * lane; i + 1u < len; i += 128u) {
@@ -1144,7 +1298,7 @@
   }
 }
 
-template <int RB>
+template <int RB, bool P32>
 __global__ __launch_bounds__(256) void k_csr_bucket(const CsrArgs a) {
   __shared__ uint32_t cnt_all[4][1u << RB];
   __shared__ uint32_t off_all[4][(1u << RB) + 1u];
@@ -1172,9 +1326,15 @@
     for (uint32_t k = 0; k < kPer; ++k) {
       if (k >= turns) { break; }
       const uint32_t j = k * 64u + lane;
-      const unsigned long long e = j < c ? a.links[start + j] : 0ull;
-      dst[k] = (uint32_t)e;
-      rowpos[k] = ((uint32_t)(e >> 32) - a.first) & (rows - 1u);
+      if constexpr (P32) {
+        const uint32_t e = j < c ? a.links32[start + j] : 0u;
+        dst[k] = e & (0xFFFFFFFFu >> a.r);
+        rowpos[k] = e >> (32u - a.r);
+      } else {
+        const unsigned long long e = j < c ? a.links[start + j] : 0ull;
+        dst[k] = (uint32_t)e;
+        rowpos[k] = ((uint32_t)(e >> 32) - a.first) & (rows - 1u);
+      }
     }
 #pragma unroll
     for (uint32_t k = 0; k < kPer; ++k) {
@@ -1214,6 +1374,7 @@
   }
 }
 
+template <bool P32>
 __global__ __launch_bounds__(256) void k_csr_bucket_big(const CsrArgs a) {
   __shared__ uint32_t cnt[1u << kCsrMaxR];
   __shared__ uint32_t off[(1u << kCsrMaxR) + 1u];
@@ -1229,7 +1390,7 @@
     const uint32_t row0 = b << a.r;
     for (uint32_t i = threadIdx.x; i < rows; i += 256u) { cnt[i] = 0u; }
     __syncthreads();
-    for (uint32_t j = threadIdx.x; j < c; j += 256u) { atomicAdd(&cnt[((uint32_t)(a.links[start + j] >> 32) - a.first) & (rows - 1u)], 1u); }
+    for (uint32_t j = threadIdx.x; j < c; j += 256u) { uint32_t row, t; csr_link<P32>(a, start + j, rows, row, t); atomicAdd(&cnt[row], 1u); }
     __syncthreads();
     {
       const uint32_t i0 = 2u * threadIdx.x, i1 = i0 + 1u;
@@ -1249,8 +1410,9 @@
     __syncthreads();
     if (c <= kCsrBigStage) {
       for (uint32_t j = threadIdx.x; j < c; j += 256u) {
-        const unsigned long long e = a.links[start + j];
-        stage[atomicAdd(&cnt[((uint32_t)(e >> 32) - a.first) & (rows - 1u)], 1u)] = (uint32_t)e;
+        uint32_t row, t;
+        csr_link<P32>(a, start + j, rows, row, t);
+        stage[atomicAdd(&cnt[row], 1u)] = t;
       }
       __syncthreads();
       sort_short_rows(stage, off, rows, threadIdx.x, 256u);
@@ -1262,8 +1424,9 @@
       for (uint32_t j = threadIdx.x; j < c; j += 256u) { if (start + j < a.cap) { a.neighbours[start + j] = stage[j]; } }
     } else if (start + c <= a.cap) {
       for (uint32_t j = threadIdx.x; j < c; j += 256u) {
-        const unsigned long long e = a.links[start + j];
-        a.neighbours[start + atomicAdd(&cnt[((uint32_t)(e >> 32) - a.first) & (rows - 1u)], 1u)] = (uint32_t)e;
+        uint32_t row, t;
+        csr_link<P32>(a, start + j, rows, row, t);
+        a.neighbours[start + atomicAdd(&cnt[row], 1u)] = t;
       }
       __threadfence();
       __syncthreads();
diff --git a/swarm_amd/csrc/swa_internal.h b/swarm_amd/csrc/swa_internal.h
--- a/swarm_amd/csrc/swa_internal.h
+++ b/swarm_amd/csrc/swa_internal.h
@@ -115,7 +115,7 @@
   uint64_t list_regions_items = 0;
   bool stream_index = false;
   uint32_t stream_extra_bits = 0;
-  swa_dbuf d_stream[30];
+  swa_dbuf d_stream[34];
   bool member_index = false, only_oversized = false;
   uint32_t over_mass = 0;
   uint64_t mtable_size = 0, mbloom_words = 0;
@@ -131,6 +131,8 @@
   int pair_blocks[4] = {};
   bool g1_lds_opt_in = false;
   bool part_lds_opt_in = false;
+  uint32_t chain_epoch = 0;
+  bool chain_scan_off = false;
   uint32_t pair_lds_opt_in = 0;
   bool csr_has_diffs = false;
   uint64_t csr_total = 0;
```
